# rojas-diego/tokengeex

Hardware: AMD Instinct MI355X
Metric: MB/s raw bytes encoded (and tokens/s) at 32K/64K vocab, 1/2/4/8 GPUs (higher is better)
Workload: dtype f64

## Files before the change

include/tgx.h:

```cpp
#ifndef TGX_H
#define TGX_H

#include <stddef.h>
#include <stdint.h>

#ifdef __cplusplus
extern "C" {
#endif

#define TGX_ABI_VERSION 1

typedef enum tgx_status {
    TGX_OK = 0,
    TGX_ERR_IO = 1,
    TGX_ERR_JSON = 2,
    TGX_ERR_TOKEN_ID_OOB = 3,
    TGX_ERR_NO_PATH = 4,
    TGX_ERR_DEVICE = 5,
    TGX_ERR_Z_NOT_NORMAL = 6,
    TGX_ERR_INVALID = 7,
    TGX_ERR_UNSUPPORTED = 8
} tgx_status;

#define TGX_MAX_TOKEN_LEN 64
// ... 229 lines not shown

double tgx_sample_u01(uint64_t seed, uint64_t sample, uint64_t pos, uint32_t len);
tgx_status tgx_encode_batch_sample(tgx_model *m, const uint8_t *text, const uint64_t *offs,
                                   uint64_t n_samples, double alpha, uint64_t seed,
                                   double *logz, tgx_result **out);
tgx_status tgx_encode_corpus_sample(tgx_model *m, tgx_corpus *c, double alpha, uint64_t seed,
                                    double *logz, tgx_result **out);

#define TGX_MAX_NBEST 16
tgx_status tgx_encode_batch_nbest(tgx_model *m, const uint8_t *text, const uint64_t *offs, uint64_t n_samples,
                                  uint32_t nbest, double *scores, uint32_t *n_found, tgx_result **out);
tgx_status tgx_encode_corpus_nbest(tgx_model *m, tgx_corpus *c, uint32_t nbest,
                                   double *scores, uint32_t *n_found, tgx_result **out);

tgx_status tgx_count_tokens(tgx_model *m, tgx_corpus *c, uint64_t *freq);

tgx_status tgx_count_pairs(tgx_model *m, tgx_corpus *c, uint64_t **keys, uint64_t **counts,
                           uint64_t *n_pairs);
tgx_status tgx_count_pairs_top(tgx_model *m, tgx_corpus *c, uint64_t max_pairs, uint64_t **keys,
                               uint64_t **counts, uint64_t *n_pairs, uint64_t *n_total);

tgx_status tgx_estep(tgx_model *m, tgx_corpus *c, uint64_t snippet_len, double dropout,
                     uint64_t seed, double *expected, double *logz_sum);

void tgx_free(void *p);
void tgx_pool_trim(int device);
void *tgx_host_alloc(uint64_t bytes);
void tgx_host_free(void *p);

double tgx_digamma(double x);
tgx_status tgx_prune_m_step(const double *expected, const uint8_t *keep, uint32_t vocab_size,
                            uint32_t *out_idx, double *out_score, uint32_t *out_n);
tgx_status tgx_prune_alternatives(const tgx_flat_trie *trie, const uint8_t *bytes, const uint64_t *offs,
                                  const double *scores, uint32_t vocab_size, uint8_t *always_keep,
                                  uint32_t *alt_offs, uint32_t **alt_ids);
tgx_status tgx_model_prune_alternatives(const tgx_model *m, uint8_t *always_keep, uint32_t *alt_offs, uint32_t **alt_ids);
tgx_status tgx_prune_select(const uint64_t *freq, const uint8_t *keep, const uint8_t *always_keep,
                            const uint32_t *alt_offs, const uint32_t *alt_ids, const double *scores,
                            uint32_t vocab_size, uint64_t n_samples, uint32_t pruned_size,
                            uint32_t *out_idx, uint32_t *out_n);

int tgx_last_kernel_times(const tgx_model *m, const char **names, float *ms, int cap);
uint64_t tgx_last_algorithmic_bytes(const tgx_model *m);
uint32_t tgx_last_encode_waves_per_cu(const tgx_model *m);
uint64_t tgx_last_encode_redo_samples(const tgx_model *m);
uint64_t tgx_last_encode_long_samples(const tgx_model *m);
uint64_t tgx_last_estep_pieces(const tgx_model *m);
uint64_t tgx_last_estep_redo(const tgx_model *m);
uint32_t tgx_last_encode_corun_cus(const tgx_model *m);
uint32_t tgx_encode_corun_timeouts(const tgx_model *m);
uint32_t tgx_model_score_values(const tgx_model *m);
uint32_t tgx_last_encode_hot_values(const tgx_model *m);
uint32_t tgx_last_encode_lean_items(const tgx_model *m);

static inline double tgx_dropout_u01(uint64_t seed, uint64_t sample, uint64_t pos, uint32_t len) {
    uint64_t x = seed ^ (sample * 0x9E3779B97F4A7C15ULL) ^ (pos * 0xC2B2AE3D27D4EB4FULL) ^
                 ((uint64_t)len * 0x165667B19E3779F9ULL);
    x ^= x >> 30;
    x *= 0xBF58476D1CE4E5B9ULL;
    x ^= x >> 27;
    x *= 0x94D049BB133111EBULL;
    x ^= x >> 31;
    return (double)(x >> 11) * (1.0 / 9007199254740992.0);
}

#ifdef __cplusplus
}
#endif
#endif
```

tokengeex_amd/_lib.py:

```python
from __future__ import annotations

import ctypes as C
import os

import numpy as np

_HERE = os.path.dirname(os.path.abspath(__file__))
LIB_PATH = os.path.join(_HERE, "libtgx.so")

OK, ERR_IO, ERR_JSON, ERR_TOKEN_ID_OOB, ERR_NO_PATH, ERR_DEVICE, ERR_Z_NOT_NORMAL, ERR_INVALID, \
    ERR_UNSUPPORTED = range(9)
MAX_TOKEN_LEN = 64
MAX_NBEST = 16
ESTEP_SNIPPET_LEN = 81920
NO_ID = 0xFFFFFFFF
LAYOUT_PAD_LEFT, LAYOUT_TRUNC_LEFT, LAYOUT_I64 = 1, 2, 4
FRONT_CRLF = 1
SPAN_CHARS = 8

_vp, _u64, _u32, _i, _d = C.c_void_p, C.c_uint64, C.c_uint32, C.c_int, C.c_double
_pvp, _pu64 = C.POINTER(C.c_void_p), C.POINTER(C.c_uint64)
SYMBOLS = {
    "tgx_last_error": (C.c_char_p, []),
    "tgx_last_error_detail": (None, [_pu64, _pu64, _pu64]),
# ... 15 lines not shown
                                     C.POINTER(C.c_double)]),
    "tgx_flat_trie_stats": (None, [_vp, _pu64, _pu64, C.POINTER(C.c_uint32)]),
    "tgx_flat_trie_copy": (None, [_vp, _vp, _vp, _vp]),
    "tgx_tok_hash_selftest": (_i, [_vp, _vp, _u32, C.POINTER(C.c_uint32), _pu64]),
    "tgx_dropout_u01_host": (_d, [_u64, _u64, _u64, _u32]),
    "tgx_encode_batch": (_i, [_vp, _vp, _vp, _u64, _d, _u64, _pvp]),
    "tgx_encode_batch_host": (_i, [_vp, _vp, _vp, _u64, _d, _u64, _vp, _u64, _vp, _pu64]),
    "tgx_encode_batch_multi": (_i, [_vp, _u32, _vp, _vp, _u64, _d, _u64, _vp, _u64, _vp, _pu64]),
    "tgx_result_num_samples": (_u64, [_vp]),
    "tgx_result_num_tokens": (_u64, [_vp]),
    "tgx_result_ids": (_vp, [_vp]),
    "tgx_result_offsets": (_vp, [_vp]),
    "tgx_result_copy_ids": (_i, [_vp, _vp, _u64]),
    "tgx_result_copy_offsets": (_i, [_vp, _vp, _u64]),
    "tgx_result_ids_device": (_vp, [_vp]),
    "tgx_result_offsets_device": (_vp, [_vp]),
    "tgx_result_free": (None, [_vp]),
    "tgx_corpus_upload": (_i, [_i, _vp, _vp, _u64, _pvp]),
    "tgx_corpus_free": (None, [_vp]),
    "tgx_corpus_num_samples": (_u64, [_vp]),
    "tgx_corpus_num_bytes": (_u64, [_vp]),
    "tgx_encode_corpus": (_i, [_vp, _vp, _d, _u64, _pvp]),
    "tgx_count_tokens": (_i, [_vp, _vp, _vp]),
    "tgx_count_pairs": (_i, [_vp, _vp, _pvp, _pvp, _pu64]),
    "tgx_count_pairs_top": (_i, [_vp, _vp, _u64, _pvp, _pvp, _pu64, _pu64]),
    "tgx_estep": (_i, [_vp, _vp, _u64, _d, _u64, _vp, C.POINTER(C.c_double)]),
    "tgx_split_specials": (_i, [_vp, _vp, _u64, _vp, _vp, _u32, _vp, _pvp, _pvp, _pvp, _pu64]),
    "tgx_pack_segments": (_i, [_vp, _vp, _vp, _vp, _u64, _i, _vp, _vp, _pu64]),
    "tgx_normalize_segments": (_i, [_u32, _vp, _vp, _vp, _u64, _pvp, _pvp]),
    "tgx_unidata_version": (C.c_char_p, []),
    "tgx_assemble_ids": (_i, [_vp, _vp, _u64, _vp, _vp, _u32, _vp, _vp]),
    "tgx_decode_batch": (_i, [_vp, _vp, _u32, _vp, _vp, _u32, _vp, _vp, _u64, _i, _pvp, _vp, _pu64, _pu64]),
    "tgx_utf8_lossy": (_u64, [_vp, _u64, _vp]),
    "tgx_substring_df": (_i, [_i, _vp, _u64, _vp, _vp, _vp, _vp, _u64, _u32, _d, _u64, _pvp, _pvp, _pvp, _pu64, _pu64, _pu64]),
    "tgx_substring_df_top": (_i, [_i, _vp, _u64, _vp, _vp, _vp, _vp, _u64, _u32, _d, _u64, _u64, _pvp, _pvp, _pvp, _pu64, _pu64, _pu64,
                                  _pu64, C.POINTER(C.c_uint32)]),
    "tgx_generate_u01": (_d, [_u64, _u64, _u64]),
    "tgx_free": (None, [_vp]),
    "tgx_pool_trim": (None, [_i]),
    "tgx_host_alloc": (_vp, [_u64]),
    "tgx_host_free": (None, [_vp]),
    "tgx_digamma": (_d, [_d]),
    "tgx_prune_m_step": (_i, [_vp, _vp, _u32, _vp, _vp, C.POINTER(C.c_uint32)]),
    "tgx_prune_alternatives": (_i, [_vp, _vp, _vp, _vp, _u32, _vp, _vp, _pvp]),
    "tgx_model_prune_alternatives": (_i, [_vp, _vp, _vp, _pvp]),
    "tgx_prune_select": (_i, [_vp, _vp, _vp, _vp, _vp, _vp, _u32, _u64, _u32, _vp, C.POINTER(C.c_uint32)]),
    "tgx_last_kernel_times": (_i, [_vp, C.POINTER(C.c_char_p), C.POINTER(C.c_float), _i]),
    "tgx_last_algorithmic_bytes": (_u64, [_vp]),
    "tgx_last_encode_waves_per_cu": (_u32, [_vp]),
    "tgx_last_encode_redo_samples": (_u64, [_vp]),
    "tgx_model_score_values": (_u32, [_vp]),
    "tgx_last_encode_hot_values": (_u32, [_vp]),
    "tgx_last_encode_lean_items": (_u32, [_vp]),
    "tgx_last_encode_long_samples": (_u64, [_vp]),
    "tgx_last_estep_pieces": (_u64, [_vp]),
    "tgx_last_estep_redo": (_u64, [_vp]),
    "tgx_last_encode_corun_cus": (_u32, [_vp]),
    "tgx_encode_corun_timeouts": (_u32, [_vp]),
    "tgx_sample_u01": (_d, [_u64, _u64, _u64, _u32]),
    "tgx_encode_batch_sample": (_i, [_vp, _vp, _vp, _u64, _d, _u64, _vp, _pvp]),
    "tgx_encode_corpus_sample": (_i, [_vp, _vp, _d, _u64, _vp, _pvp]),
    "tgx_encode_batch_nbest": (_i, [_vp, _vp, _vp, _u64, _u32, _vp, _vp, _pvp]),
    "tgx_encode_corpus_nbest": (_i, [_vp, _vp, _u32, _vp, _vp, _pvp]),
    "tgx_result_device": (_i, [_vp]),
    "tgx_result_layout_info": (_i, [_vp, _u32, _u32, _pu64, _pu64]),
    "tgx_result_pad_device": (_i, [_vp, _u32, _u32, _u32, _u32, _u32, _vp, _vp, _vp, _vp, _pu64]),
    "tgx_result_pack_device": (_i, [_vp, _u32, _u32, _u32, _u32, _u32, _vp, _vp, _vp, _vp, _pu64]),
    "tgx_layout_pad_host": (_i, [_vp, _vp, _u64, _u32, _u32, _u32, _u32, _u32, _vp, _vp, _vp, _pu64]),
    "tgx_layout_pack_host": (_i, [_vp, _vp, _u64, _u32, _u32, _u32, _u32, _u32, _vp, _vp, _vp, _pu64]),
    "tgx_assemble_result": (_i, [_vp, _vp, _vp, _vp, _u64, _u32, _pvp]),
    "tgx_result_vocab_size": (_u32, [_vp]),
    "tgx_assemble_host": (_i, [_vp, _vp, _u64, _vp, _vp, _u64, _u32, _u32, _vp, _u64, _vp]),
    "tgx_decode_result": (_i, [_vp, _vp, _vp, _vp, _u32, _i, _vp, _pvp, _pu64, _pu64]),
    "tgx_decode_padded": (_i, [_vp, _vp, _u64, _u64, _u32, _vp, _vp, _u32, _vp, _vp, _u32, _i, _vp, _pvp, _pu64, _pu64]),
    "tgx_text_num_rows": (_u64, [_vp]),
    "tgx_text_num_bytes": (_u64, [_vp]),
    "tgx_text_num_replaced": (_u64, [_vp]),
    "tgx_text_device": (_i, [_vp]),
    "tgx_text_copy_bytes": (_i, [_vp, _vp, _u64]),
    "tgx_text_copy_offsets": (_i, [_vp, _vp, _u64]),
    "tgx_text_bytes_device": (_vp, [_vp]),
    "tgx_text_offsets_device": (_vp, [_vp]),
    "tgx_text_free": (None, [_vp]),
    "tgx_corpus_from_text": (_i, [_vp, _pvp]),
    "tgx_decode_rows_host": (_i, [_vp, _vp, _u32, _vp, _vp, _u32, _vp, _u32, _vp, _u64, _u64, _vp, _vp, _u32, _i, _pvp, _vp, _pu64,
                                  _pu64, _pu64]),
    "tgx_result_spans_device": (_i, [_vp, _vp, _vp, _vp, _u32, _u32, _vp, _vp]),
    "tgx_result_pad_spans_device": (_i, [_vp, _vp, _vp, _vp, _u32, _u32, _u32, _u32, _u32, _vp, _vp]),
    "tgx_spans_host": (_i, [_vp, _vp, _u32, _vp, _vp, _u32, _vp, _vp, _u64, _u32, _u32, _u32, _u32, _vp]),
    "tgx_result_window_info": (_i, [_vp, _u32, _u32, _u32, _u32, _u32, _pu64]),
    "tgx_result_window_pad_device": (_i, [_vp, _u32, _u32, _u32, _u32, _u32, _u32, _vp, _u64, _vp, _vp, _vp, _vp, _vp]),
    "tgx_result_window_spans_device": (_i, [_vp, _vp, _vp, _vp, _u32, _u32, _u32, _u32, _u32, _u32, _vp, _u64, _vp]),
    "tgx_layout_windows_host": (_i, [_vp, _vp, _u64, _u32, _u32, _u32, _u32, _u32, _u32, _u64, _vp, _vp, _vp, _vp, _vp, _pu64]),
    "tgx_window_spans_host": (_i, [_vp, _vp, _u32, _vp, _vp, _u32, _vp, _vp, _u64, _u32, _u32, _u32, _u32, _u32, _u64, _vp, _pu64]),
    "tgx_corpus_split_specials": (_i, [_vp, _vp, _vp, _u32, _u32, _pvp, _pvp]),
    "tgx_plan_num_samples": (_u64, [_vp]),
    "tgx_plan_num_segments": (_u64, [_vp]),
    "tgx_plan_num_encoded": (_u64, [_vp]),
    "tgx_plan_device": (_i, [_vp]),
    "tgx_plan_copy": (_i, [_vp, _vp, _u64, _vp, _u64]),
    "tgx_plan_free": (None, [_vp]),
    "tgx_assemble_result_plan": (_i, [_vp, _vp, _vp, _u32, _pvp]),
    "tgx_front_last_times": (_i, [C.POINTER(C.c_char_p), C.POINTER(C.c_float), _i]),
    "tgx_corpus_copy_text": (_i, [_vp, _vp, _u64]),
    "tgx_corpus_copy_offsets": (_i, [_vp, _vp, _u64]),
    "tgx_front_host": (_i, [_vp, _vp, _u64, _vp, _vp, _u32, _u32, _vp, _pvp, _pu64, _pvp, _pvp, _pu64]),
# ... 1042 lines not shown
        ka = np.ctypeslib.as_array(C.cast(keys, C.POINTER(C.c_uint64)), shape=(max(k, 1),))[:k].copy()
        ca = np.ctypeslib.as_array(C.cast(counts, C.POINTER(C.c_uint64)), shape=(max(k, 1),))[:k].copy()
        lib.tgx_free(keys)
        lib.tgx_free(counts)
        return ka, ca, tot.value

    def estep(self, corpus: NativeCorpus, snippet_len: int = ESTEP_SNIPPET_LEN, dropout: float = 0.0,
              seed: int = 0, expected: np.ndarray | None = None) -> tuple[np.ndarray, float]:
        if expected is None:
            expected = np.zeros(self.vocab_size, np.float64)
        assert expected.dtype == np.float64 and expected.shape[0] == self.vocab_size
        z = C.c_double()
        check(lib.tgx_estep(self._h, corpus._h, snippet_len, float(dropout), seed & (2**64 - 1),
                            ptr(expected), C.byref(z)))
        return expected, z.value

    def common_prefix_search(self, s: bytes) -> list[tuple[int, int]]:
        buf = np.frombuffer(s, dtype=np.uint8)
        cap = len(s) + 1
        ids, lens = np.zeros(cap, np.uint32), np.zeros(cap, np.uint32)
        cnt = C.c_uint64()
        check(lib.tgx_common_prefix_search(self._h, ptr(buf) if len(s) else None, len(s), ptr(ids),
                                           ptr(lens), cap, C.byref(cnt)))
        return [(int(ids[i]), int(lens[i])) for i in range(cnt.value)]

    def last_kernel_times(self) -> dict[str, float]:
        names = (C.c_char_p * 8)()
        ms = (C.c_float * 8)()
        n = lib.tgx_last_kernel_times(self._h, names, ms, 8)
        return {names[i].decode(): float(ms[i]) for i in range(n)}

    def last_algorithmic_bytes(self) -> int:
        return lib.tgx_last_algorithmic_bytes(self._h)

    def last_encode_waves_per_cu(self) -> int:
        return lib.tgx_last_encode_waves_per_cu(self._h)

    def last_encode_redo_samples(self) -> int:
        return lib.tgx_last_encode_redo_samples(self._h)

    def score_values(self) -> int:
        return lib.tgx_model_score_values(self._h)

    def last_encode_hot_values(self) -> int:
        return lib.tgx_last_encode_hot_values(self._h)

    def last_encode_lean_items(self) -> tuple[int, int]:
        v = lib.tgx_last_encode_lean_items(self._h)
        return v & 0xFF, (v >> 8) & 0xFF

    def last_encode_lean_step(self) -> bool:
        return bool(self.last_encode_lean_items()[0] & 1)

    def last_encode_long_samples(self) -> int:
        return lib.tgx_last_encode_long_samples(self._h)

    def last_estep_pieces(self) -> int:
        return lib.tgx_last_estep_pieces(self._h)

    def last_estep_redo(self) -> int:
        return lib.tgx_last_estep_redo(self._h)

    def last_encode_corun_cus(self) -> int:
        return lib.tgx_last_encode_corun_cus(self._h)

    def encode_corun_timeouts(self) -> int:
        return lib.tgx_encode_corun_timeouts(self._h)


class FlatTrie:

    def __init__(self, tokens: list[bytes], scores):
        flat, offs = pack(tokens)
        sc = np.ascontiguousarray(scores, dtype=np.float64)
        h = C.c_void_p()
        check(lib.tgx_flat_trie_build(ptr(flat) if flat.size else None, ptr(offs), ptr(sc), len(tokens),
                                      C.byref(h)))
        self._h = h
        self._flat, self._offs, self._sc = flat, offs, sc

    def common_prefix_search8(self, s: bytes, max_hot: int = 6600):
        buf = np.frombuffer(s, dtype=np.uint8)
        cap = len(s) + 1
        ids, lens = np.zeros(cap, np.uint32), np.zeros(cap, np.uint32)
        nh, nc, cov = C.c_uint32(), C.c_uint64(), C.c_double()
        k = lib.tgx_flat_trie_search8(self._h, ptr(self._flat) if self._flat.size else None, ptr(self._offs), ptr(self._sc),
                                      max_hot, ptr(buf) if len(s) else None, len(s), ptr(ids), ptr(lens), cap,
                                      C.byref(nh), C.byref(nc), C.byref(cov))
        if k == 2**64 - 1:
            raise TokenGeeXError("8-byte records need fewer than 2^23 slots")
        return [(int(ids[i]), int(lens[i])) for i in range(k)], {"n_hot": nh.value, "n_cold": nc.value, "hot_coverage": cov.value}

    def __del__(self):
        if getattr(self, "_h", None):
            lib.tgx_flat_trie_free(self._h)
            self._h = None

    def common_prefix_search(self, s: bytes) -> list[tuple[int, int]]:
        buf = np.frombuffer(s, dtype=np.uint8)
        cap = len(s) + 1
        ids, lens = np.zeros(cap, np.uint32), np.zeros(cap, np.uint32)
        k = lib.tgx_flat_trie_search(self._h, ptr(buf) if len(s) else None, len(s), ptr(ids), ptr(lens), cap)
        return [(int(ids[i]), int(lens[i])) for i in range(k)]

    def stats(self) -> dict:
        a, b, c = C.c_uint64(), C.c_uint64(), C.c_uint32()
# ... 88 lines not shown
```

tokengeex_amd/build.py:

```python
from __future__ import annotations

import os
import shutil
import subprocess
import sys

HERE = os.path.dirname(os.path.abspath(__file__))
CSRC = os.path.join(HERE, "csrc")
OUT = os.path.join(HERE, "libtgx.so")
SOURCES = ["kernels.hip", "estep.hip", "encode2.hip", "encode4l.hip", "encode5.hip", "estep4.hip", "estep4l.hip", "estep7.hip", "cuts.hip", "pairs.hip", "generate.hip", "sample.hip", "nbest.hip", "layout.hip", "assemble.hip", "fim.hip", "decode.hip", "spans.hip", "front.hip", "norm.hip", "tgx_api.cpp", "host_twins.cpp", "trie_build.cpp", "prune_host.cpp", "frontback.cpp", "unicode_norm.cpp"]
HEADERS = ["api_internal.h", "kernels.h", "sample.h", "nbest.h", "layout.h", "assemble.h", "fim.h", "decode.h", "spans.h", "front.h", "norm.h", "device_common.h", "lean_gate.h", "trace_body.h", "trie_build.h", "unicode_tables.h", os.path.join("..", "..", "include", "tgx.h")]
ARCH = "gfx950"


def _hipcc() -> str:
    for cand in (os.environ.get("HIPCC"), shutil.which("hipcc"), "/opt/rocm/bin/hipcc"):
        if cand and os.path.exists(cand):
            return cand
    raise RuntimeError("hipcc not found")


def needs_build() -> bool:
    if not os.path.exists(OUT):
        return True
    t = os.path.getmtime(OUT)
    deps = [os.path.join(CSRC, f) for f in SOURCES + HEADERS] + [os.path.abspath(__file__)]
    return any(os.path.getmtime(d) > t for d in deps)


SYNTH_OUT = os.path.join(HERE, "libtgx_synth.so")


def build_synth(force: bool = False) -> str:
    src = os.path.join(CSRC, "synth_gen.c")
    if not force and os.path.exists(SYNTH_OUT) and os.path.getmtime(SYNTH_OUT) >= os.path.getmtime(src):
        return SYNTH_OUT
    subprocess.check_call(["gcc", "-O2", "-std=c11", "-fPIC", "-shared", "-o", SYNTH_OUT + ".tmp", src, "-lm"])
    os.replace(SYNTH_OUT + ".tmp", SYNTH_OUT)
    return SYNTH_OUT


FAST_OUT = os.path.join(HERE, "_tgxfast.so")


def build_pyfast(force: bool = False) -> str:
    import sysconfig
    src = os.path.join(CSRC, "pyfast.c")
    if not force and os.path.exists(FAST_OUT) and os.path.getmtime(FAST_OUT) >= os.path.getmtime(src):
        return FAST_OUT
    inc = sysconfig.get_paths()["include"]
    subprocess.check_call(["gcc", "-O2", "-std=c11", "-fPIC", "-shared", "-pthread", "-I", inc, "-o", FAST_OUT + ".tmp", src])
    os.replace(FAST_OUT + ".tmp", FAST_OUT)
    return FAST_OUT


def build(force: bool = False, verbose: bool = False) -> str:
    from concurrent.futures import ThreadPoolExecutor
    build_synth(force)
    build_pyfast(force)
    if not force and not needs_build():
        return OUT
    objdir = os.path.join(CSRC, "build")
    os.makedirs(objdir, exist_ok=True)
    hdr_time = max(os.path.getmtime(os.path.join(CSRC, h)) for h in HEADERS)
# ... 33 lines not shown
```

tokengeex_amd/csrc/device_common.h:

```cpp
#pragma once
#include <hip/hip_runtime.h>
#include <stdint.h>

namespace tgx {

__device__ __forceinline__ uint32_t readlane_u32(uint32_t v, uint32_t lane) {
    return (uint32_t)__builtin_amdgcn_readlane((int)v, (int)lane);
}
__device__ __forceinline__ uint64_t readlane_u64(uint64_t v, uint32_t lane) {
    uint32_t lo = readlane_u32((uint32_t)v, lane);
    uint32_t hi = readlane_u32((uint32_t)(v >> 32), lane);
    return ((uint64_t)hi << 32) | lo;
}
__device__ __forceinline__ double readlane_f64(double v, uint32_t lane) {
    return __longlong_as_double((long long)readlane_u64((uint64_t)__double_as_longlong(v), lane));
}
__device__ __forceinline__ uint64_t first_u64(uint64_t v) {
    uint32_t lo = (uint32_t)__builtin_amdgcn_readfirstlane((int)(uint32_t)v);
    uint32_t hi = (uint32_t)__builtin_amdgcn_readfirstlane((int)(uint32_t)(v >> 32));
    return ((uint64_t)hi << 32) | lo;
}
__device__ __forceinline__ uint64_t rotl64(uint64_t x, uint32_t r) {
    r &= 63u;
    return (x << r) | (x >> ((64u - r) & 63u));
// ... 98 lines not shown
    return ((uint64_t)hi << 32) | lo;
}

__device__ __forceinline__ uint64_t claim_rows(unsigned long long* queue, bool need_new, uint32_t r) {
    const uint64_t want = __builtin_amdgcn_ballot_w64(need_new) & kRowLane0;
    uint64_t k = ~0ull;
    if (want != 0) {
        const uint64_t base = wave_fetch_add(queue, (uint32_t)__builtin_popcountll(want));
        if (need_new) k = base + (uint64_t)__builtin_popcountll(want & ((1ull << (r * 16u)) - 1ull));
    }
    return k;
}

__device__ __forceinline__ uint64_t claim_rows_chunk(unsigned long long* queue, bool need_new, uint32_t r, uint32_t chunk) {
    const uint64_t want = __builtin_amdgcn_ballot_w64(need_new) & kRowLane0;
    uint64_t k = ~0ull;
    if (want != 0) {
        const uint64_t base = wave_fetch_add(queue, (uint32_t)__builtin_popcountll(want) * chunk);
        if (need_new) k = base + (uint64_t)__builtin_popcountll(want & ((1ull << (r * 16u)) - 1ull)) * chunk;
    }
    return k;
}

__device__ __forceinline__ uint4 load_rec(const uint4* __restrict__ trie, uint32_t t) {
    uint4 r = trie[t];
    asm volatile("" : "+v"(r.x), "+v"(r.y), "+v"(r.z), "+v"(r.w));
    return r;
}

__device__ __forceinline__ uint64_t bp8_base(uint64_t beg, uint32_t s) { return (beg + 128ull * s) & ~3ull; }
__device__ __forceinline__ uint32_t bp8_perm(uint32_t j) { return (j & ~63u) | ((j & 15u) << 2) | ((j >> 4) & 3u); }


constexpr uint32_t kNoStep = 0xFFu;

template <int U>
__device__ __forceinline__ void relax4_step(double sv, double& acc, uint32_t& bpv, uint32_t& fin, uint32_t& fhi) {
    constexpr uint64_t MU = kRowLane0 << U;
    const double best = row_bcast_f64<U>(acc);
    fin = sel_u32(MU, bpv, fin);
    fhi = sel_u32(MU, (uint32_t)((uint64_t)__double_as_longlong(acc) >> 32), fhi);
    const double cand = best + sv;
    const uint64_t take = __builtin_amdgcn_fcmp(cand, acc, 2 ) | MU;
    acc = sel_f64(take, cand, acc);
    bpv = sel_imm_u32<U>(take, bpv);
}

constexpr int kLeanStep = 1, kLeanBcast = 2, kLeanFetch = 4;
constexpr uint32_t kLeanResetHi = 0xFFEFFFFFu;
constexpr uint32_t kLeanUnreachedHi = 0xFFE00000u;
template <int LN>
__device__ __forceinline__ bool relax5_reached(uint32_t fhi) { return (LN & kLeanStep) ? fhi < kLeanUnreachedHi : fhi != 0xFFF00000u; }

template <int U, int LN = 0>
__device__ __forceinline__ void relax5_step(double sv, double& acc, uint32_t& bpv, uint32_t& fin, uint32_t& fhi) {
    constexpr uint64_t MU = kRowLane0 << U;
    double best;
    if constexpr ((LN & kLeanBcast) != 0) best = row_bcast_f64_b<U>(acc);
    else best = row_bcast_f64<U>(acc);
    fin = sel_u32(MU, bpv, fin);
    fhi = sel_u32(MU, (uint32_t)((uint64_t)__double_as_longlong(acc) >> 32), fhi);
    const double acc_r = sel_f64(MU, -__builtin_huge_val(), acc);
    const double cand = best + sv;
    const uint64_t take = __builtin_amdgcn_fcmp(cand, acc_r, 2 );
    asm("v_max_f64 %0, %1, %2" : "=v"(acc) : "v"(acc_r), "v"(cand));
    bpv = sel_imm_u32<U>(take, bpv);
}

template <int U, int LN>
__device__ __forceinline__ void relax5_lean_step(double sv, double& acc, uint32_t& bpv, uint32_t& fin) {
    constexpr uint64_t MU = kRowLane0 << U;
    double best;
    if constexpr ((LN & kLeanBcast) != 0) best = row_bcast_f64_b<U>(acc);
    else best = row_bcast_f64<U>(acc);
    fin = sel_u32(MU, bpv, fin);
    const uint64_t ab = (uint64_t)__double_as_longlong(acc);
    const uint32_t hi_r = sel_u32(MU, kLeanResetHi, (uint32_t)(ab >> 32));
    const double acc_r = __hiloint2double((int)hi_r, (int)(uint32_t)ab);
    const double cand = best + sv;
    const uint64_t take = __builtin_amdgcn_fcmp(cand, acc_r, 2 );
    asm("v_max_f64 %0, %1, %2" : "=v"(acc) : "v"(acc_r), "v"(cand));
    bpv = sel_imm_u32<U>(take, bpv);
}


__device__ __forceinline__ uint32_t rotl32_dev(uint32_t x, int r) { return __builtin_rotateleft32(x, (uint32_t)r); }
__device__ __forceinline__ uint64_t tok_hash64_dev(uint32_t w0, uint32_t w1, uint32_t w2, uint32_t w3, uint32_t len, uint32_t seed) {
    uint32_t a = (w0 ^ (len << 27) ^ seed) * 0x85EBCA6Bu;
    a ^= a >> 15;
    uint32_t b = a;
    a = (a + w1) * 0xC2B2AE35u;
    a ^= a >> 13;
    b = rotl32_dev(b, 11) ^ a;
    a = (a + w2) * 0x27D4EB2Fu;
    a ^= a >> 16;
    b = rotl32_dev(b, 11) ^ a;
    a = (a + w3) * 0x165667B1u;
    a ^= a >> 15;
    b = rotl32_dev(b, 11) + (w0 ^ rotl32_dev(w1, 8) ^ rotl32_dev(w2, 16) ^ rotl32_dev(w3, 24));
    return ((uint64_t)b << 32) | a;
}


__device__ __forceinline__ uint64_t tok_hash64_long_dev(const uint32_t* w, uint32_t len, uint32_t seed) {
    uint32_t a = (w[0] ^ (len << 27) ^ seed) * 0x85EBCA6Bu;
    a ^= a >> 15;
    uint32_t b = a;
    a = (a + w[1]) * 0xC2B2AE35u;
    a ^= a >> 13;
    b = rotl32_dev(b, 11) ^ a;
    a = (a + w[2]) * 0x27D4EB2Fu;
    a ^= a >> 16;
    b = rotl32_dev(b, 11) ^ a;
    a = (a + w[3]) * 0x165667B1u;
    a ^= a >> 15;
    b = rotl32_dev(b, 11) + (w[0] ^ rotl32_dev(w[1], 8) ^ rotl32_dev(w[2], 16) ^ rotl32_dev(w[3], 24));
    if (len > 16u) {
        a = (a + w[4]) * 0x85EBCA6Bu;
        a ^= a >> 15;
        b = rotl32_dev(b, 11) ^ a;
        a = (a + w[5]) * 0xC2B2AE35u;
        a ^= a >> 13;
        b = rotl32_dev(b, 11) ^ a;
        a = (a + w[6]) * 0x27D4EB2Fu;
        a ^= a >> 16;
        b = rotl32_dev(b, 11) ^ a;
        a = (a + w[7]) * 0x165667B1u;
        a ^= a >> 15;
        b = rotl32_dev(b, 11) + (w[4] ^ rotl32_dev(w[5], 8) ^ rotl32_dev(w[6], 16) ^ rotl32_dev(w[7], 24));
    }
    return ((uint64_t)b << 32) | a;
}


__device__ __forceinline__ int row_max_exponent(double acc) {
// ... 20 lines not shown
```

tokengeex_amd/csrc/encode5.hip:

```cpp
#include <hip/hip_runtime.h>
#include <stdint.h>

#include <type_traits>

#include "device_common.h"
#include "kernels.h"

namespace tgx {

constexpr uint32_t kE5RowStride = 512;
constexpr uint32_t kE5GroupBytes = 4 * kE5RowStride;

template <int PPL>
struct WalkCtx {
    __amdgpu_buffer_rsrc_t trie;
    uint32_t s, l32;
    double dropout;
    uint64_t seed;
    bool estep_rule = false;
};

struct Res5 {
    __amdgpu_buffer_rsrc_t cold;
    uint32_t tab;
// ... 223 lines not shown
    fval = sel_f64(MU, acc, fval);
    const double best = row_bcast_f64<U>(acc);
    const double cur = sel_f64(MU, far, acc);
    const uint32_t curbp = sel_u32(MU, fbp, bpv);
    far = sel_f64(MU, -__builtin_huge_val(), far);
    const double cand = best + sv;
    const uint64_t take = __builtin_amdgcn_fcmp(cand, cur, 2 );
    asm("v_max_f64 %0, %1, %2" : "=v"(acc) : "v"(cur), "v"(cand));
    bpv = sel_imm_u32<U>(take, curbp);
}

template <bool DROPOUT>
__device__ __forceinline__ void e5_long_tail(__amdgpu_buffer_rsrc_t trie, const uint8_t* __restrict__ text16, uint32_t rec_x, bool alive,
                                             uint32_t maxd, uint32_t lane, uint32_t g, uint32_t list_off, double dropout, uint64_t seed,
                                             uint32_t s, uint32_t pg) {
    bool more = alive && maxd > 16u;
    if (__builtin_amdgcn_ballot_w64(more) == 0) return;
    struct __attribute__((packed, aligned(1))) Bytes16 { uint32_t w[4]; };
    Bytes16 b{{0u, 0u, 0u, 0u}};
    if (more) b = *reinterpret_cast<const Bytes16*>(text16);
    uint32_t x = rec_x;
#pragma unroll 1
    for (uint32_t d = 16u; d < 32u; ++d) {
        more = more && d < maxd;
        if (__builtin_amdgcn_ballot_w64(more) == 0) break;
        const uint32_t bi = d - 16u;
        const uint32_t word = (bi & 8u) ? ((bi & 4u) ? b.w[3] : b.w[2]) : ((bi & 4u) ? b.w[1] : b.w[0]);
        const uint32_t c = (word >> ((bi & 3u) * 8u)) & 0xFFu;
        const uint2 rec = buf_ld8(trie, more ? ((x ^ (c << 3)) & 0xFFFFFFu) : 0u);
        more = more && (rec.x >> 24) == c;
        const uint32_t rank = rec.y & 0xFFFFu;
        bool term = more && rank != 0u;
        if (DROPOUT) {
            if (term) term = dropout < dropout_u01(seed, s, pg, d + 1u);
        }
        if (term) {
            const uint32_t slot = __hip_atomic_fetch_add((__attribute__((address_space(3))) uint32_t*)(uintptr_t)list_off, 1u, __ATOMIC_RELAXED, __HIP_MEMORY_SCOPE_WORKGROUP);
            if (slot < kE5LongCap) lds_st<uint32_t>(list_off + 8u + slot * 4u, lane | (g << 6) | (d << 8) | (rank << 16));
        }
        x = rec.x;
    }
}

#define E5_STAMP(i)                                                    \
    if (P.stamps) {                                                    \
        __builtin_amdgcn_sched_barrier(0);                             \
        const uint64_t _now = (uint64_t)__builtin_amdgcn_s_memtime(); \
        __builtin_amdgcn_s_waitcnt(0xC07F);                            \
        __builtin_amdgcn_sched_barrier(0);                             \
        seg[i] += _now - t_last;                                       \
        t_last = _now;                                                 \
    }

template <bool DROPOUT, bool COLD, int PPL, bool LONG, int CK = 0, int LN = 0>
__global__ __launch_bounds__(1024, (PPL == 1 ? 8 : (PPL == 2 ? 6 : (PPL == 3 ? 4 : 1)))) void encode5_kernel(EncodeParams P, Encode5Params Q) {
    static_assert(!LONG || PPL == 4, "the long-token build runs four positions per lane");
    static_assert(LN == 0 || (!LONG && !DROPOUT), "the long-token and dropout builds keep the kernel as it was");
    extern __shared__ __align__(16) unsigned char smem[];
    constexpr uint32_t LM = LONG ? 32 : 16;
    constexpr uint32_t SPAN = 16u * PPL;
    const uint32_t lane = threadIdx.x & 63u;
    const uint32_t l = lane & 15u, r = lane >> 4;
    const uint32_t wave = threadIdx.x >> 6;
    const uint2* __restrict__ trie = reinterpret_cast<const uint2*>(Q.trie8);
    const __amdgpu_buffer_rsrc_t trie_b = make_rsrc(Q.trie8, Q.trie_bytes);
    const uint32_t lds0 = (uint32_t)reinterpret_cast<uintptr_t>(smem);
    double* const score_tab = reinterpret_cast<double*>(smem);
    const uint32_t hot_bytes = 8u * (Q.n_hot + 1u);
    const __amdgpu_buffer_rsrc_t values = make_rsrc(reinterpret_cast<const unsigned char*>(Q.values) + hot_bytes, 8u * (Q.n_values - Q.n_hot));
    const uint2* rootc = reinterpret_cast<const uint2*>(smem + Q.root_off);
    unsigned char* wbase = smem + Q.idx_off + (size_t)wave * (PPL * kE5GroupBytes);
    {
        for (uint32_t i = threadIdx.x; i <= Q.n_hot; i += blockDim.x) score_tab[i] = Q.values[i];
        uint2* rw = reinterpret_cast<uint2*>(smem + Q.root_off);
        for (uint32_t i = threadIdx.x; i < 256u; i += blockDim.x) rw[i] = trie[(Q.root_base & ~255u) + i];
        if (Q.started && threadIdx.x == 0u) __hip_atomic_fetch_add(Q.started, 1u, __ATOMIC_RELAXED, __HIP_MEMORY_SCOPE_SYSTEM);
        __syncthreads();
    }
    const __amdgpu_buffer_rsrc_t cold_values = values;

    uint32_t s = 0, n = 0, p0 = 0;
    uint64_t beg = 0;
    bool live = false, need_new = true;
    const double ninf = -__builtin_huge_val();
    double acc = ninf, far = ninf;
    uint32_t bpv = kNoStep, fbp = kFarCode;
    bool redo = false;
    uint32_t wn[4 * PPL + 1];
    uint32_t pk = 0, pk_j = 0;
    bool pk_dirty = false;
#pragma unroll
    for (int q = 0; q <= 4 * PPL; ++q) wn[q] = 0;
    const uint32_t my_col = r * kE5RowStride + ((l - 1u) & 15u) * 32u;
    const uint32_t wbase_off = lds0 + Q.idx_off + wave * (PPL * kE5GroupBytes);
    const uint32_t wr_off = wbase_off + r * kE5RowStride + l * 2u;
    const uint32_t col_off = wbase_off + my_col;
    const uint32_t list_off = lds0 + Q.list_off + wave * ((kE5LongBytes + 15u) & ~15u);
    uint64_t seg[5] = {0, 0, 0, 0, 0};
    uint64_t t_last = P.stamps ? (uint64_t)__builtin_amdgcn_s_memtime() : 0;
    uint32_t iters = 0;

    uint64_t local_next = 0, local_end = 0;
    for (;;) {
        {
            uint64_t k = ~0ull;
            const bool have_local = need_new && local_next < local_end;
            if (have_local) k = local_next++;
            const uint64_t kc = claim_rows_chunk(P.queue, need_new && !have_local, r, Q.claim_chunk);
            if (need_new && !have_local) {
                k = kc;
// ... 120 lines not shown
                    n_list = (uint32_t)__builtin_amdgcn_readfirstlane((int)lds_ld<uint32_t>(list_off));
                    slow = n_list != 0u || __builtin_amdgcn_ballot_w64((uint32_t)((uint64_t)__double_as_longlong(far) >> 32) != 0xFFF00000u) != 0;
                }
                if (LONG && slow) {
                    auto rank_of = [&](int u) { return (u & 1) ? (cw[u >> 1] >> 16) : (cw[u >> 1] & 0xFFFFu); };
                    double fval = ninf;
                    relax5l_step<0>(e5_score_one<COLD>(lds0, cold_values, rank_of(0), hot_bytes), acc, bpv, far, fbp, fin[g], fval);
                    relax5l_step<1>(e5_score_one<COLD>(lds0, cold_values, rank_of(1), hot_bytes), acc, bpv, far, fbp, fin[g], fval);
                    relax5l_step<2>(e5_score_one<COLD>(lds0, cold_values, rank_of(2), hot_bytes), acc, bpv, far, fbp, fin[g], fval);
                    relax5l_step<3>(e5_score_one<COLD>(lds0, cold_values, rank_of(3), hot_bytes), acc, bpv, far, fbp, fin[g], fval);
                    relax5l_step<4>(e5_score_one<COLD>(lds0, cold_values, rank_of(4), hot_bytes), acc, bpv, far, fbp, fin[g], fval);
                    relax5l_step<5>(e5_score_one<COLD>(lds0, cold_values, rank_of(5), hot_bytes), acc, bpv, far, fbp, fin[g], fval);
                    relax5l_step<6>(e5_score_one<COLD>(lds0, cold_values, rank_of(6), hot_bytes), acc, bpv, far, fbp, fin[g], fval);
                    relax5l_step<7>(e5_score_one<COLD>(lds0, cold_values, rank_of(7), hot_bytes), acc, bpv, far, fbp, fin[g], fval);
                    relax5l_step<8>(e5_score_one<COLD>(lds0, cold_values, rank_of(8), hot_bytes), acc, bpv, far, fbp, fin[g], fval);
                    relax5l_step<9>(e5_score_one<COLD>(lds0, cold_values, rank_of(9), hot_bytes), acc, bpv, far, fbp, fin[g], fval);
                    relax5l_step<10>(e5_score_one<COLD>(lds0, cold_values, rank_of(10), hot_bytes), acc, bpv, far, fbp, fin[g], fval);
                    relax5l_step<11>(e5_score_one<COLD>(lds0, cold_values, rank_of(11), hot_bytes), acc, bpv, far, fbp, fin[g], fval);
                    relax5l_step<12>(e5_score_one<COLD>(lds0, cold_values, rank_of(12), hot_bytes), acc, bpv, far, fbp, fin[g], fval);
                    relax5l_step<13>(e5_score_one<COLD>(lds0, cold_values, rank_of(13), hot_bytes), acc, bpv, far, fbp, fin[g], fval);
                    relax5l_step<14>(e5_score_one<COLD>(lds0, cold_values, rank_of(14), hot_bytes), acc, bpv, far, fbp, fin[g], fval);
                    relax5l_step<15>(e5_score_one<COLD>(lds0, cold_values, rank_of(15), hot_bytes), acc, bpv, far, fbp, fin[g], fval);
                    const uint32_t cnt = n_list < kE5LongCap ? n_list : kE5LongCap;
#pragma unroll 1
                    for (uint32_t i = 0; i < cnt; ++i) {
                        const uint32_t e = (uint32_t)__builtin_amdgcn_readfirstlane((int)lds_ld<uint32_t>(list_off + 8u + i * 4u));
                        if (((e >> 6) & 3u) != (uint32_t)g) continue;
                        const uint32_t src = e & 63u, d = (e >> 8) & 31u;
                        const double score = e5_score_one<COLD>(lds0, cold_values, e >> 16, hot_bytes);
                        const double cand = readlane_f64(fval, src) + score;
                        const uint32_t tt = (src & 15u) + d + 1u;
                        const bool mine = (lane >> 4) == (src >> 4) && l == (tt & 15u);
                        const bool to_far = tt >= 32u;
                        const double curv = to_far ? far : acc;
                        const uint32_t curc = to_far ? fbp : bpv;
                        const bool longer = !(curc & kFarCode) || d > (curc & 31u);
                        const bool take = mine && (cand > curv || (cand == curv && longer));
                        if (take && to_far) {
                            far = cand;
                            fbp = kFarCode | d;
                        }
                        if (take && !to_far) {
                            acc = cand;
                            bpv = kFarCode | d;
                        }
                    }
                    reached[g] = fval > ninf;
                    if (g + 1 < PPL) {
                        load_iw(g + 1, nw);
                        if (!COLD) e5_scores_issue<4>(lds0, nw, 0, sa);
                    }
                    continue;
                }
                if constexpr (LN == 0) {
                    if (COLD) {
                        double sv[8], sw[8];
                        e5_scores_cold<8>(lds0, cold_values, cw, 0, hot_bytes, sv);
                        e5_scores_cold<8>(lds0, cold_values, cw, 8, hot_bytes, sw);
                        if (g + 1 < PPL) load_iw(g + 1, nw);
                        relax5_step<0>(sv[0], acc, bpv, fin[g], fhi);
                        relax5_step<1>(sv[1], acc, bpv, fin[g], fhi);
                        relax5_step<2>(sv[2], acc, bpv, fin[g], fhi);
                        relax5_step<3>(sv[3], acc, bpv, fin[g], fhi);
                        relax5_step<4>(sv[4], acc, bpv, fin[g], fhi);
                        relax5_step<5>(sv[5], acc, bpv, fin[g], fhi);
                        relax5_step<6>(sv[6], acc, bpv, fin[g], fhi);
                        relax5_step<7>(sv[7], acc, bpv, fin[g], fhi);
                        relax5_step<8>(sw[0], acc, bpv, fin[g], fhi);
                        relax5_step<9>(sw[1], acc, bpv, fin[g], fhi);
                        relax5_step<10>(sw[2], acc, bpv, fin[g], fhi);
                        relax5_step<11>(sw[3], acc, bpv, fin[g], fhi);
                        relax5_step<12>(sw[4], acc, bpv, fin[g], fhi);
                        relax5_step<13>(sw[5], acc, bpv, fin[g], fhi);
                        relax5_step<14>(sw[6], acc, bpv, fin[g], fhi);
                        relax5_step<15>(sw[7], acc, bpv, fin[g], fhi);
                    } else {
                        e5_scores_issue<4>(lds0, cw, 4, sb);
                        if (g + 1 < PPL) load_iw(g + 1, nw);
                        relax5_step<0>(e5_score_value(sa[0]), acc, bpv, fin[g], fhi);
                        relax5_step<1>(e5_score_value(sa[1]), acc, bpv, fin[g], fhi);
                        relax5_step<2>(e5_score_value(sa[2]), acc, bpv, fin[g], fhi);
                        relax5_step<3>(e5_score_value(sa[3]), acc, bpv, fin[g], fhi);
                        e5_scores_issue<4>(lds0, cw, 8, sa);
                        relax5_step<4>(e5_score_value(sb[0]), acc, bpv, fin[g], fhi);
                        relax5_step<5>(e5_score_value(sb[1]), acc, bpv, fin[g], fhi);
                        relax5_step<6>(e5_score_value(sb[2]), acc, bpv, fin[g], fhi);
                        relax5_step<7>(e5_score_value(sb[3]), acc, bpv, fin[g], fhi);
                        e5_scores_issue<4>(lds0, cw, 12, sb);
                        relax5_step<8>(e5_score_value(sa[0]), acc, bpv, fin[g], fhi);
                        relax5_step<9>(e5_score_value(sa[1]), acc, bpv, fin[g], fhi);
                        relax5_step<10>(e5_score_value(sa[2]), acc, bpv, fin[g], fhi);
                        relax5_step<11>(e5_score_value(sa[3]), acc, bpv, fin[g], fhi);
                        if (g + 1 < PPL) e5_scores_issue<4>(lds0, nw, 0, sa);
                        relax5_step<12>(e5_score_value(sb[0]), acc, bpv, fin[g], fhi);
                        relax5_step<13>(e5_score_value(sb[1]), acc, bpv, fin[g], fhi);
                        relax5_step<14>(e5_score_value(sb[2]), acc, bpv, fin[g], fhi);
                        relax5_step<15>(e5_score_value(sb[3]), acc, bpv, fin[g], fhi);
                    }
                    reached[g] = fhi != 0xFFF00000u;
                } else {
                    const bool full = !(LN & kLeanStep) || ((end_groups >> g) & 1u) != 0u;
#define E5_STEP(U, SV)                                                   \
        if (FULL) relax5_step<U, LN>(SV, acc, bpv, fin[g], fhi);              \
        else relax5_lean_step<U, LN>(SV, acc, bpv, fin[g]);
                    auto steps = [&](auto full_tag) {
                        constexpr bool FULL = decltype(full_tag)::value;
                        if (COLD) {
                            double sv[8], sw[8];
                            e5_scores_cold<8, LN>(lds0, cold_values, cw, 0, hot_bytes, sv);
                            e5_scores_cold<8, LN>(lds0, cold_values, cw, 8, hot_bytes, sw);
                            if (g + 1 < PPL) load_iw(g + 1, nw);
                            E5_STEP(0, sv[0]) E5_STEP(1, sv[1]) E5_STEP(2, sv[2]) E5_STEP(3, sv[3])
                            E5_STEP(4, sv[4]) E5_STEP(5, sv[5]) E5_STEP(6, sv[6]) E5_STEP(7, sv[7])
                            E5_STEP(8, sw[0]) E5_STEP(9, sw[1]) E5_STEP(10, sw[2]) E5_STEP(11, sw[3])
                            E5_STEP(12, sw[4]) E5_STEP(13, sw[5]) E5_STEP(14, sw[6]) E5_STEP(15, sw[7])
                        } else {
                            e5_scores_issue<4, LN>(lds0, cw, 4, sb);
                            if (g + 1 < PPL) load_iw(g + 1, nw);
                            E5_STEP(0, e5_score_value(sa[0])) E5_STEP(1, e5_score_value(sa[1]))
                            E5_STEP(2, e5_score_value(sa[2])) E5_STEP(3, e5_score_value(sa[3]))
                            e5_scores_issue<4, LN>(lds0, cw, 8, sa);
                            E5_STEP(4, e5_score_value(sb[0])) E5_STEP(5, e5_score_value(sb[1]))
                            E5_STEP(6, e5_score_value(sb[2])) E5_STEP(7, e5_score_value(sb[3]))
                            e5_scores_issue<4, LN>(lds0, cw, 12, sb);
                            E5_STEP(8, e5_score_value(sa[0])) E5_STEP(9, e5_score_value(sa[1]))
                            E5_STEP(10, e5_score_value(sa[2])) E5_STEP(11, e5_score_value(sa[3]))
                            if (g + 1 < PPL) e5_scores_issue<4, LN>(lds0, nw, 0, sa);
                            E5_STEP(12, e5_score_value(sb[0])) E5_STEP(13, e5_score_value(sb[1]))
                            E5_STEP(14, e5_score_value(sb[2])) E5_STEP(15, e5_score_value(sb[3]))
                        }
                    };
                    if (full) steps(std::true_type{});
                    else steps(std::false_type{});
#undef E5_STEP
                    reached[g] = !full || relax5_reached<LN>(fhi);
                }
            }
        } else {
#pragma unroll
            for (int g = 0; g < PPL; ++g) {
                fin[g] = kNoStep;
                reached[g] = true;
            }
        }
        __builtin_amdgcn_wave_barrier();
        if (!(P.flags & 32u)) __builtin_amdgcn_s_setprio(2);
        E5_STAMP(3)

        uint8_t* const bpw = P.bp8 + bp8_base(beg, s);
#pragma unroll
        for (int g = 0; g < PPL; ++g)
            if (live && pg[g] >= 1u && pg[g] <= n) {
                const uint32_t b = reached[g] ? (LONG ? e5_winner_len_m1(fin[g], l) : ((l - fin[g] - 1u) & 15u)) : 0xFFu;
                const uint32_t j = pg[g] - 1u, kq = (j >> 4) & 3u;
                pk = (kq == 0u) ? b : (pk | (b << (8u * kq)));
                pk_j = j;
                pk_dirty = true;
                if (kq == 3u) {
                    __builtin_nontemporal_store(pk, reinterpret_cast<uint32_t*>(bpw + (bp8_perm(j) & ~3u)));
                    pk_dirty = false;
                }
            }
        if (LONG) {
            const uint32_t n_all = (uint32_t)__builtin_amdgcn_readfirstlane((int)lds_ld<uint32_t>(list_off));
            if (n_all > kE5LongCap) {
                if (live && !redo && l == 0u) P.redo_list[atomicAdd(P.redo_count, 1ULL)] = s;
                redo = true;
            }
        }
        if (live && n - p0 < SPAN && pk_dirty) {
            __builtin_nontemporal_store(pk, reinterpret_cast<uint32_t*>(bpw + (bp8_perm(pk_j) & ~3u)));
            pk_dirty = false;
        }
        if (live) {
            const uint32_t left = n - p0;
            if (left < SPAN) {
#pragma unroll
                for (int g = 0; g < PPL; ++g)
                    if (left == 16u * g + l) P.status[s] = (n == 0u || reached[g]) ? 1u : 0u;
                need_new = true;
            } else {
                p0 += SPAN;
            }
        }
        E5_STAMP(4)
    }
    if (P.stamps && lane == 0) {
        unsigned long long* o = P.stamps + (size_t)(blockIdx.x * (blockDim.x >> 6) + wave) * 8u;
        for (int i = 0; i < 5; ++i) o[i] = seg[i];
        o[5] = iters;
    }
}

constexpr uint32_t kE6Walkers = 3;
constexpr uint32_t kE6Slots = kE6Walkers + 2u;
struct E6Ctrl {
    uint32_t epoch;
    uint32_t s, n, trip0;
    uint64_t beg;
    uint32_t relax_done;
    uint32_t pad_;
    uint32_t walk_done[8];
    uint32_t ack[4];
    uint32_t pool_used[8];
    uint32_t pad2_[4];
};
constexpr uint32_t kE6Done = 0xFFFFFFFFu;

__device__ __forceinline__ uint32_t lds_load(const uint32_t* p) { return __hip_atomic_load(p, __ATOMIC_RELAXED, __HIP_MEMORY_SCOPE_WORKGROUP); }
__device__ __forceinline__ void lds_store(uint32_t* p, uint32_t v) { __hip_atomic_store(p, v, __ATOMIC_RELAXED, __HIP_MEMORY_SCOPE_WORKGROUP); }

template <bool COLD, int LN = 0>
__device__ __forceinline__ void e6_load_quarter(uint32_t tab, __amdgpu_buffer_rsrc_t cold, uint32_t hot_bytes,
                                                const uint32_t (&iw)[8], int q, double (&sv)[4]) {
    if (COLD) {
        e5_scores_cold<4, LN>(tab, cold, iw, 4 * q, hot_bytes, sv);
    } else {
        u32x2_t sp[4];
        e5_scores_issue<4, LN>(tab, iw, 4 * q, sp);
#pragma unroll
        for (int u = 0; u < 4; ++u) sv[u] = e5_score_value(sp[u]);
    }
}

template <bool DROPOUT, bool COLD, int LN = 0>
__global__ __launch_bounds__(64 * (1 + 4 * kE6Walkers), 8) void encode6_kernel(EncodeParams P, Encode5Params Q) {
    static_assert(LN == 0 || !DROPOUT, "the dropout builds keep the kernel as it was");
    static_assert((LN & (kLeanStep | kLeanBcast)) == 0, "encode6_kernel: the score fetch only (the lean step spills here)");
    extern __shared__ __align__(16) unsigned char smem[];
    constexpr uint32_t LM = 16;
    constexpr uint32_t K = kE6Walkers, G = kE6Slots;
    const uint32_t lane = threadIdx.x & 63u;
// ... 418 lines not shown
        if (live) {
            if (n - p0 < SPAN) need_new = true;
            else p0 += SPAN;
        }
    }
    if (zsum != 0.0) atomicAdd(P.logz_sum, zsum);
}

typedef void (*estep5_fn)(Estep4Params, Encode5Params);
static estep5_fn pick_estep5(bool dropout, bool cold, int ppl) {
#define TGX_E5F(D, C)                                                                        \
    (ppl == 1 ? estep5_fwd_kernel<D, C, 1> : ppl == 2 ? estep5_fwd_kernel<D, C, 2> : ppl == 3 ? estep5_fwd_kernel<D, C, 3> : estep5_fwd_kernel<D, C, 4>)
    if (dropout) return cold ? TGX_E5F(true, true) : TGX_E5F(true, false);
    return cold ? TGX_E5F(false, true) : TGX_E5F(false, false);
#undef TGX_E5F
}
hipError_t estep5_waves_per_simd(bool dropout, bool cold, int ppl, int* out) {
    hipFuncAttributes attr;
    hipError_t e = hipFuncGetAttributes(&attr, reinterpret_cast<const void*>(pick_estep5(dropout, cold, ppl)));
    if (e != hipSuccess) return e;
    const int regs = (attr.numRegs + 7) & ~7;
    *out = regs > 0 ? (512 / regs > 8 ? 8 : 512 / regs) : 8;
    return hipSuccess;
}
hipError_t launch_estep5_fwd(const Estep4Params& p, Encode5Params q, bool cold, int ppl, int waves, uint32_t blocks, hipStream_t stream) {
    const uint32_t lds = encode5_lds_layout(q.n_hot, false, waves, ppl, &q.list_off, &q.root_off, &q.idx_off);
    if (lds > 160u * 1024u || q.n_hot > q.n_values || (!cold && q.n_hot != q.n_values) || ppl < 1 || ppl > 4) return hipErrorInvalidValue;
    estep5_fn fn = pick_estep5(p.dropout > 0.0, cold, ppl);
    hipError_t e = hipFuncSetAttribute(reinterpret_cast<const void*>(fn), hipFuncAttributeMaxDynamicSharedMemorySize, 160 * 1024);
    if (e != hipSuccess) return e;
    hipLaunchKernelGGL(fn, dim3(blocks), dim3(64u * (uint32_t)waves), lds, stream, p, q);
    return hipGetLastError();
}

typedef void (*encode5_fn)(EncodeParams, Encode5Params);
#ifdef TGX_E5_LEAN_ITEMS
constexpr int kE5LeanHot = TGX_E5_LEAN_ITEMS, kE5LeanCold = TGX_E5_LEAN_ITEMS, kE5LeanCold3 = TGX_E5_LEAN_ITEMS;
constexpr int kE6Lean = kLeanFetch;
#else
constexpr int kE5LeanHot = kLeanFetch;
constexpr int kE5LeanCold = kLeanFetch;
constexpr int kE5LeanCold3 = kLeanStep | kLeanBcast | kLeanFetch;
constexpr int kE6Lean = kLeanFetch;
#endif
static_assert(kE5LeanHot > 0 && kE5LeanHot <= 7 && kE5LeanCold > 0 && kE5LeanCold <= 7 && kE5LeanCold3 > 0 && kE5LeanCold3 <= 7,
              "a mask of kLeanStep, kLeanBcast, kLeanFetch");
constexpr int lean_without_step(int items) { return items & ~kLeanStep; }
bool encode5_has_lean(bool dropout, bool long_tokens) { return !dropout && !long_tokens; }
int encode5_lean_items(bool cold, int ppl, bool step_ok) {
    const int items = cold ? (ppl == 3 ? kE5LeanCold3 : kE5LeanCold) : kE5LeanHot;
    return step_ok ? items : lean_without_step(items);
}
int encode6_lean_items() { return kE6Lean; }
static encode5_fn pick_encode5(bool dropout, bool cold, int ppl, bool long_tokens, int compact, bool lean, bool step_ok) {
    if (long_tokens) {
        if (cold) return dropout ? encode5_kernel<true, true, 4, true> : encode5_kernel<false, true, 4, true>;
        return dropout ? encode5_kernel<true, false, 4, true> : encode5_kernel<false, false, 4, true>;
    }
    if (dropout) {
        if (cold) {
            if (ppl == 1) return encode5_kernel<true, true, 1, false>;
            if (ppl == 2) return encode5_kernel<true, true, 2, false>;
            if (ppl == 3) return encode5_kernel<true, true, 3, false>;
            return encode5_kernel<true, true, 4, false>;
        }
        if (ppl == 1) return encode5_kernel<true, false, 1, false>;
        if (ppl == 2) return encode5_kernel<true, false, 2, false>;
        if (ppl == 3) return encode5_kernel<true, false, 3, false>;
        return encode5_kernel<true, false, 4, false>;
    }
#define TGX_E5K(C, PL, LN) \
    (compact == 4 ? encode5_kernel<false, C, PL, false, 4, LN> : compact == 5 ? encode5_kernel<false, C, PL, false, 5, LN> \
     : compact == 6 ? encode5_kernel<false, C, PL, false, 6, LN> : compact == 7 ? encode5_kernel<false, C, PL, false, 7, LN> \
     : compact == 8 ? encode5_kernel<false, C, PL, false, 8, LN> : encode5_kernel<false, C, PL, false, 0, LN>)
#define TGX_E5L(LNH, LNC, LNC3) \
    if (cold) { \
        if (ppl == 1) return encode5_kernel<false, true, 1, false, 0, LNC>; \
        if (ppl == 2) return TGX_E5K(true, 2, LNC); \
        if (ppl == 3) return TGX_E5K(true, 3, LNC3); \
        return TGX_E5K(true, 4, LNC); \
    } \
    if (ppl == 1) return encode5_kernel<false, false, 1, false, 0, LNH>; \
    if (ppl == 2) return TGX_E5K(false, 2, LNH); \
    if (ppl == 3) return TGX_E5K(false, 3, LNH); \
    return TGX_E5K(false, 4, LNH);
    if (lean && step_ok) {
        TGX_E5L(kE5LeanHot, kE5LeanCold, kE5LeanCold3)
    }
    if (lean) {
        TGX_E5L(lean_without_step(kE5LeanHot), lean_without_step(kE5LeanCold), lean_without_step(kE5LeanCold3))
    }
    TGX_E5L(0, 0, 0)
#undef TGX_E5L
#undef TGX_E5K
}

uint32_t encode5_lds_layout(uint32_t n_hot, bool long_tokens, int waves, int ppl, uint32_t* list_off, uint32_t* root_off, uint32_t* idx_off) {
    const uint32_t lo = (8u * (n_hot + 1u) + 15u) & ~15u;
    const uint32_t score_bytes = lo + (long_tokens ? (uint32_t)waves * ((kE5LongBytes + 15u) & ~15u) : 0u);
    if (list_off) *list_off = lo;
    const uint32_t ro = (score_bytes + 15u) & ~15u;
    const uint32_t io = (ro + 2048u + 511u) & ~511u;
    if (root_off) *root_off = ro;
    if (idx_off) *idx_off = io;
    return io + (uint32_t)waves * (uint32_t)ppl * kE5GroupBytes;
}
uint32_t encode5_max_hot(bool long_tokens, int waves, int ppl, uint32_t budget) {
    const uint32_t fixed = encode5_lds_layout(0u, long_tokens, waves, ppl, nullptr, nullptr, nullptr) + 512u;
    return budget > fixed + 64u ? (budget - fixed) / 8u : 0u;
}

hipError_t encode5_waves_per_simd(bool dropout, bool cold, int ppl, bool long_tokens, int compact, bool lean, bool step_ok, int* out) {
    hipFuncAttributes attr;
    hipError_t e = hipFuncGetAttributes(&attr, reinterpret_cast<const void*>(pick_encode5(dropout, cold, ppl, long_tokens, compact, lean && encode5_has_lean(dropout, long_tokens), step_ok)));
    if (e != hipSuccess) return e;
    const int regs = (attr.numRegs + 7) & ~7;
    *out = regs > 0 ? (512 / regs > 8 ? 8 : 512 / regs) : 8;
    return hipSuccess;
}

uint32_t encode6_lds_layout(uint32_t n_hot, uint32_t pool, uint32_t* root_off, uint32_t* ctrl_off, uint32_t* ring_off) {
    const uint32_t score_bytes = 8u * (1u + 4u * kE6Slots * pool + n_hot);
    const uint32_t ro = (score_bytes + 15u) & ~15u;
    const uint32_t co = ro + 2048u;
    const uint32_t go = (co + 4u * (uint32_t)sizeof(E6Ctrl) + 511u) & ~511u;
    if (root_off) *root_off = ro;
    if (ctrl_off) *ctrl_off = co;
    if (ring_off) *ring_off = go;
    return go + 4u * kE6Slots * kE5GroupBytes;
}
uint32_t encode6_pool_total(uint32_t pool) { return 4u * kE6Slots * pool; }
uint32_t encode6_max_hot(uint32_t budget, uint32_t pool) {
    const uint32_t fixed = encode6_lds_layout(0u, pool, nullptr, nullptr, nullptr) + 512u;
    return budget > fixed + 64u ? (budget - fixed) / 8u : 0u;
}
static hipError_t lean_lds_check(const void* fn) {
    hipFuncAttributes attr;
    const hipError_t e = hipFuncGetAttributes(&attr, fn);
    if (e != hipSuccess) return e;
    return attr.sharedSizeBytes == 0 ? hipSuccess : hipErrorInvalidValue;
}

hipError_t launch_encode6(const EncodeParams& p, Encode5Params q, bool cold, bool lean, uint32_t blocks, hipStream_t stream) {
    q.ring_slots = kE6Slots;
    if (!cold) q.pool = 0u;
    const uint32_t lds = encode6_lds_layout(q.n_hot, q.pool, &q.root_off, &q.ctrl_off, &q.ring_off);
    if (lds > 160u * 1024u || q.n_hot > q.n_values || (!cold && q.n_hot != q.n_values) ||
        (uint64_t)q.n_values + 4ull * kE6Slots * q.pool > 65535ull)
        return hipErrorInvalidValue;
    lean = lean && encode5_has_lean(p.dropout > 0.0, false);
    auto fn = cold ? (p.dropout > 0.0 ? encode6_kernel<true, true> : lean ? encode6_kernel<false, true, kE6Lean> : encode6_kernel<false, true>)
                   : (p.dropout > 0.0 ? encode6_kernel<true, false> : lean ? encode6_kernel<false, false, kE6Lean> : encode6_kernel<false, false>);
    hipError_t e = hipFuncSetAttribute(reinterpret_cast<const void*>(fn), hipFuncAttributeMaxDynamicSharedMemorySize, 160 * 1024);
    if (e != hipSuccess) return e;
    if (lean && (e = lean_lds_check(reinterpret_cast<const void*>(fn))) != hipSuccess) return e;
    hipLaunchKernelGGL(fn, dim3(blocks), dim3(64u * (1u + 4u * kE6Walkers)), lds, stream, p, q);
    return hipGetLastError();
}

hipError_t launch_encode5(const EncodeParams& p, Encode5Params q, bool cold, int ppl, bool long_tokens, int compact, bool lean, bool step_ok,
                          int waves, uint32_t blocks, uint32_t min_lds, hipStream_t stream) {
    uint32_t lds = encode5_lds_layout(q.n_hot, long_tokens, waves, ppl, &q.list_off, &q.root_off, &q.idx_off);
    if (lds > 160u * 1024u || q.n_hot > q.n_values || (!cold && q.n_hot != q.n_values) || (long_tokens && ppl != 4) ||
        (compact != 0 && (compact < 4 || compact > 8)))
        return hipErrorInvalidValue;
    lean = lean && encode5_has_lean(p.dropout > 0.0, long_tokens);
    encode5_fn fn = pick_encode5(p.dropout > 0.0, cold, ppl, long_tokens, compact, lean, step_ok);
    hipError_t e = hipFuncSetAttribute(reinterpret_cast<const void*>(fn), hipFuncAttributeMaxDynamicSharedMemorySize, 160 * 1024);
    if (e != hipSuccess) return e;
    if (lean && (e = lean_lds_check(reinterpret_cast<const void*>(fn))) != hipSuccess) return e;
    if (lds < min_lds && min_lds <= 160u * 1024u) lds = min_lds;
    hipLaunchKernelGGL(fn, dim3(blocks), dim3(64u * (uint32_t)waves), lds, stream, p, q);
    return hipGetLastError();
}

}
```

tokengeex_amd/csrc/kernels.h:

```cpp
#pragma once
#include <hip/hip_runtime.h>
#include <stdint.h>

#include "decode.h"
#include "fim.h"
#include "spans.h"

namespace tgx {

constexpr uint32_t kTraceStride = 2;

struct EncodeParams {
    const uint8_t* text;
    const uint64_t* offs;
    const uint32_t* order;
    uint64_t n_samples;
    const void* trie;
    const uint32_t* tokid;
    uint32_t root_base;
    uint32_t n_slots;
    uint32_t lm;
    uint32_t* bp;
    uint32_t* tmp;
    uint32_t* counts;
// ... 184 lines not shown
    uint32_t n_slots;
    uint32_t root_base;
    const double* wtab;
    uint32_t n_tok, n_hot;
    double* expected;
    double* zsnip;
    double* logz_sum;
    unsigned long long* range_flag;
    unsigned long long* queue;
    double* alpha;
    int32_t* aexp;
    unsigned char* mscratch;
    double dropout;
    uint64_t seed;
    uint32_t root_off, zero_off, idx_off;
};
uint32_t estep7_redo_max_hot(bool wide);
hipError_t launch_estep7_redo(Estep7RedoParams p, bool wide, uint32_t num_cus, hipStream_t stream);
uint32_t estep7_lds_layout(uint32_t n_hot, bool wide, int waves, int ppl, uint32_t* root_off, uint32_t* zero_off, uint32_t* idx_off);
uint32_t estep7_max_hot(bool wide, int waves, int ppl, uint32_t budget);
hipError_t estep7_waves_per_simd(bool dropout, bool cold, bool wide, int ppl, int* out);
hipError_t launch_estep7(Estep7Params p, bool wide, int ppl, int waves, uint32_t blocks, hipStream_t stream);
hipError_t launch_match_count(const uint8_t* text, uint64_t n_bytes, uint32_t chunk, uint64_t stride, const void* trie8t, uint32_t n_slots,
                              uint32_t root_base, uint32_t n_tok, unsigned int* counts, uint32_t num_cus, hipStream_t stream);
hipError_t launch_value_count(const uint8_t* text, uint64_t n_bytes, uint32_t chunk, uint64_t stride, const void* trie8, uint32_t n_slots,
                              uint32_t root_base, uint32_t n_values, uint32_t max_len, unsigned int* counts, uint32_t num_cus, hipStream_t stream);
hipError_t launch_rank_remap(void* trie8t, uint32_t n_slots, const uint32_t* perm, hipStream_t stream);
hipError_t launch_snip_z_check(const double* zsnip, uint64_t n_snips, unsigned long long* err_snip, hipStream_t stream);
hipError_t launch_piece_z_add(const double* zarr, const uint32_t* psnip, const uint32_t* order, uint64_t n_order, double* zsnip, hipStream_t stream);

hipError_t estep4_prepare();
hipError_t launch_estep4_fwd(const Estep4Params& p, uint32_t num_cus, hipStream_t stream);
hipError_t launch_estep4_bwd(const Estep4Params& p, uint32_t num_cus, hipStream_t stream);
hipError_t estep4l_prepare();
hipError_t launch_estep4l_fwd(const Estep4Params& p, int ppl, bool long_tokens, uint32_t num_cus, hipStream_t stream);
hipError_t launch_estep4l_bwd(const Estep4Params& p, int ppl, bool long_tokens, uint32_t num_cus, uint32_t groups_wanted, hipStream_t stream);
hipError_t launch_estep4_reduce(const double* rep, double* out, uint32_t n_slots, uint32_t n_replicas,
                                hipStream_t stream);

uint32_t estep_lds_bytes_per_block(uint32_t lm);
uint32_t estep_waves_per_block(uint32_t lm);
hipError_t estep_max_blocks_per_cu(uint32_t lm, int* out);
hipError_t launch_estep(const EstepParams& p, uint32_t blocks, hipStream_t stream);

uint32_t encode_lds_bytes_per_block(uint32_t lm);
uint32_t encode_waves_per_block(uint32_t lm);
hipError_t encode_max_blocks_per_cu(uint32_t lm, int* out);
hipError_t launch_encode(const EncodeParams& p, uint32_t blocks, hipStream_t stream);
uint32_t encode4_group_bytes();
hipError_t encode4_waves_per_simd(bool dropout, int ppl, bool root, int* out);
hipError_t launch_encode4(const EncodeParams& p, int ppl, int waves, uint32_t blocks, bool root, hipStream_t stream);
uint32_t encode4_lds_bytes(int waves, int ppl, bool root);
hipError_t launch_trace(const EncodeParams& p, uint32_t blocks, hipStream_t stream);
uint32_t encode5_lds_layout(uint32_t n_hot, bool long_tokens, int waves, int ppl, uint32_t* list_off, uint32_t* root_off, uint32_t* idx_off);
uint32_t encode5_max_hot(bool long_tokens, int waves, int ppl, uint32_t budget);
bool encode5_has_lean(bool dropout, bool long_tokens);
int encode5_lean_items(bool cold, int ppl, bool step_ok);
int encode6_lean_items();
hipError_t encode5_waves_per_simd(bool dropout, bool cold, int ppl, bool long_tokens, int compact, bool lean, bool step_ok, int* out);
uint32_t encode6_lds_layout(uint32_t n_hot, uint32_t pool, uint32_t* root_off, uint32_t* ctrl_off, uint32_t* ring_off);
uint32_t encode6_max_hot(uint32_t budget, uint32_t pool);
uint32_t encode6_pool_total(uint32_t pool);
hipError_t estep5_waves_per_simd(bool dropout, bool cold, int ppl, int* out);
hipError_t launch_estep5_fwd(const struct Estep4Params& p, Encode5Params q, bool cold, int ppl, int waves, uint32_t blocks, hipStream_t stream);
hipError_t launch_encode6(const EncodeParams& p, Encode5Params q, bool cold, bool lean, uint32_t blocks, hipStream_t stream);
hipError_t launch_encode5(const EncodeParams& p, Encode5Params q, bool cold, int ppl, bool long_tokens, int compact, bool lean, bool step_ok,
                          int waves, uint32_t blocks, uint32_t min_lds, hipStream_t stream);
hipError_t launch_encode2(const EncodeParams& p, uint32_t num_cus, bool permuted, hipStream_t stream);
hipError_t launch_trace32(const EncodeParams& p, uint32_t blocks, bool permuted, hipStream_t stream);
hipError_t launch_encode4l(const EncodeParams& p, uint32_t num_cus, hipStream_t stream);
hipError_t scan_temp_bytes(uint64_t n, size_t* bytes);
hipError_t launch_scan(uint32_t* counts, uint64_t* offsets, uint64_t n, void* temp, size_t temp_bytes, hipStream_t stream);
hipError_t launch_compact(const CompactParams& p, uint32_t blocks, bool rows, hipStream_t stream);

struct LayoutParams {
    const uint32_t* ids;
    const uint64_t* offs;
    uint64_t n_rows;
    uint32_t len;
    uint32_t pad, bos, eos;
    uint32_t flags;
    void* out;
    uint8_t* mask;
    int32_t* lengths;
    int32_t* doc;
    int32_t* pos;
    unsigned long long* counter;
};
hipError_t launch_layout_max_row(const uint64_t* offs, uint64_t n_rows, unsigned long long* max_out, hipStream_t stream);
hipError_t launch_layout_pad(const LayoutParams& p, hipStream_t stream);
hipError_t launch_layout_pack(const LayoutParams& p, uint64_t n_stream, uint64_t n_out, hipStream_t stream);
struct WindowParams {
    LayoutParams base;
    const uint64_t* wo;
    uint32_t stride;
    int32_t* window_row;
    int32_t* window_first;
};
hipError_t launch_layout_window_count(const uint64_t* offs, uint64_t n_rows, uint32_t room, uint32_t step, uint32_t* counts,
                                      unsigned long long* max_out, hipStream_t stream);
hipError_t launch_layout_windows(const WindowParams& q, uint64_t n_windows, hipStream_t stream);

struct AssembleParams {
    const uint32_t* ids;
    const uint64_t* offs;
    const uint64_t* seg_offs;
    const int32_t* seg_special;
    uint64_t* rank;
    uint64_t* starts;
    uint64_t n_segs, n_samples;
    uint64_t n_out;
    uint32_t vocab_size;
    uint32_t* out_ids;
    uint64_t* out_offs;
};
hipError_t assemble_scan_temp_bytes(uint64_t n_segs, size_t* bytes);
hipError_t launch_assemble_ranks(int32_t* seg_special, uint64_t* rank, uint64_t n_segs, void* temp, size_t temp_bytes, hipStream_t stream);
hipError_t launch_assemble_starts(const AssembleParams& p, hipStream_t stream);
hipError_t launch_assemble_fill(const AssembleParams& p, hipStream_t stream);
// ... 64 lines not shown
```

tokengeex_amd/csrc/kernels.hip:

```cpp
#include <hip/hip_runtime.h>
#include <stdint.h>

#include <rocprim/device/device_scan.hpp>
#include <rocprim/iterator/transform_iterator.hpp>

#include "kernels.h"
#include "trace_body.h"
#include "device_common.h"

namespace tgx {

struct WaveCtx {
    const uint4* __restrict__ trie;
    uint32_t root_base;
    double dropout;
    uint64_t seed;
    bool use_dropout;
    uint32_t flags;
};

__device__ __forceinline__ void block_generic(const WaveCtx& C, const uint8_t* __restrict__ text, uint32_t n,
                                              uint32_t s, uint32_t p0, uint32_t lane, uint32_t LM,
                                              double* sc, uint32_t* hl, uint8_t* txt, uint32_t* __restrict__ bp,
                                              double& acc, uint32_t& bpv, uint64_t& reach, uint32_t& reach_n) {
// ... 424 lines not shown
            relax5_step<6>(sv[6], acc, bpv, fin[g], fhi);
            relax5_step<7>(sv[7], acc, bpv, fin[g], fhi);
            relax5_step<8>(sv[8], acc, bpv, fin[g], fhi);
            relax5_step<9>(sv[9], acc, bpv, fin[g], fhi);
            relax5_step<10>(sv[10], acc, bpv, fin[g], fhi);
            relax5_step<11>(sv[11], acc, bpv, fin[g], fhi);
            relax5_step<12>(sv[12], acc, bpv, fin[g], fhi);
            relax5_step<13>(sv[13], acc, bpv, fin[g], fhi);
            relax5_step<14>(sv[14], acc, bpv, fin[g], fhi);
            relax5_step<15>(sv[15], acc, bpv, fin[g], fhi);
            reached[g] = fhi != 0xFFF00000u;
        }
        __builtin_amdgcn_wave_barrier();
        TGX_STAMP(3)

        uint8_t* const bpw = P.bp8 + bp8_base(beg, s);
#pragma unroll
        for (int g = 0; g < PPL; ++g)
            if (live && pg[g] >= 1u && pg[g] <= n) {
                const uint32_t b = reached[g] ? ((l - fin[g] - 1u) & 15u) : 0xFFu;
                const uint32_t j = pg[g] - 1u, kq = (j >> 4) & 3u;
                pk = (kq == 0u) ? b : (pk | (b << (8u * kq)));
                pk_j = j;
                pk_dirty = true;
                if (kq == 3u) {
                    __builtin_nontemporal_store(pk, reinterpret_cast<uint32_t*>(bpw + (bp8_perm(j) & ~3u)));
                    pk_dirty = false;
                }
            }
        if (live && n - p0 < SPAN && pk_dirty) {
            __builtin_nontemporal_store(pk, reinterpret_cast<uint32_t*>(bpw + (bp8_perm(pk_j) & ~3u)));
            pk_dirty = false;
        }
        if (live) {
            const uint32_t left = n - p0;
            if (left < SPAN) {
#pragma unroll
                for (int g = 0; g < PPL; ++g)
                    if (left == 16u * g + l) P.status[s] = (n == 0u || reached[g]) ? 1u : 0u;
                need_new = true;
            } else {
                p0 += SPAN;
            }
        }
        TGX_STAMP(4)
    }
    if (STAMP && lane == 0 && P.stamps) {
        unsigned long long* o = P.stamps + (size_t)(blockIdx.x * wpb + wave) * 8u;
        for (int i = 0; i < 5; ++i) o[i] = seg[i];
        o[5] = iters;
    }
}

template <bool STAMP, bool CARRY, int K>
__global__ __launch_bounds__(256) void trace_kernel(EncodeParams P) {
    __shared__ typename TraceRingEntry<CARRY>::type ring_all[4][kTraceRing];
    trace_body<16, true, STAMP, CARRY, K>(P, ring_all[threadIdx.x >> 6]);
}

__global__ __launch_bounds__(1024) void scan_counts_kernel(const uint32_t* __restrict__ counts,
                                                           uint64_t* __restrict__ offsets,
                                                           uint64_t n) {
    __shared__ uint64_t wsum[16];
    __shared__ uint64_t carry_s;
    constexpr uint32_t E = 8;
    const uint32_t tid = threadIdx.x, lane = tid & 63u, wave = tid >> 6;
    if (tid == 0) carry_s = 0;
    __syncthreads();
    for (uint64_t base = 0; base < n; base += 1024u * E) {
        const uint64_t i0 = base + (uint64_t)tid * E;
        uint32_t c[E];
        uint64_t v = 0;
#pragma unroll
        for (uint32_t e = 0; e < E; ++e) {
            c[e] = (i0 + e < n) ? counts[i0 + e] : 0u;
            v += c[e];
        }
        uint64_t x = v;
        for (int off = 1; off < 64; off <<= 1) {
            uint64_t y = __shfl_up(x, off);
            if ((int)lane >= off) x += y;
        }
        if (lane == 63) wsum[wave] = x;
        __syncthreads();
        uint64_t wprefix = 0;
        for (uint32_t w = 0; w < wave; ++w) wprefix += wsum[w];
        const uint64_t carry = carry_s;
        uint64_t run = carry + wprefix + x - v;
#pragma unroll
        for (uint32_t e = 0; e < E; ++e) {
            if (i0 + e < n) offsets[i0 + e] = run;
            run += c[e];
        }
        __syncthreads();
        if (tid == 1023) carry_s = run;
        __syncthreads();
    }
    if (tid == 0) offsets[n] = carry_s;
}

template <bool ROWS>
__global__ __launch_bounds__(256) void compact_kernel(CompactParams P) {
    const uint32_t lane = threadIdx.x & 63u;
    const uint32_t sub = ROWS ? (lane & 15u) : lane, width = ROWS ? 16u : 64u;
    const uint64_t n_units = (uint64_t)gridDim.x * 4u * (ROWS ? 4u : 1u);
    const uint32_t wave_id = blockIdx.x * 4u + (threadIdx.x >> 6);
    for (uint64_t k = ROWS ? (uint64_t)wave_id * 4u + (lane >> 4) : (uint64_t)wave_id; k < P.n_samples; k += n_units) {
        const uint32_t s = ROWS ? (uint32_t)k : P.order[k];
        const uint64_t end = P.offs[s + 1];
        const uint64_t o0 = P.out_offs[s];
// ... 32 lines not shown
}

hipError_t launch_encode(const EncodeParams& p, uint32_t blocks, hipStream_t stream) {
    const uint32_t lds = encode_lds_bytes_per_block(p.lm);
    const dim3 block(64u * encode_waves_per_block(p.lm));
    hipLaunchKernelGGL(pick_kernel(p.lm), dim3(blocks), block, lds, stream, p);
    return hipGetLastError();
}

hipError_t encode_max_blocks_per_cu(uint32_t lm, int* out) {
    const uint32_t lds = encode_lds_bytes_per_block(lm);
    const int threads = (int)(64u * encode_waves_per_block(lm));
    if (lds > 160u * 1024u) return hipErrorInvalidValue;
    encode_fn fn = pick_kernel(lm);
    hipError_t e = hipFuncSetAttribute(reinterpret_cast<const void*>(fn),
                                       hipFuncAttributeMaxDynamicSharedMemorySize, (int)lds);
    if (e != hipSuccess) return e;
    return hipOccupancyMaxActiveBlocksPerMultiprocessor(out, fn, threads, lds);
}

typedef void (*encode4_fn)(EncodeParams);
static encode4_fn pick_encode4(bool dropout, int ppl, bool stamp, bool root) {
    if (stamp) return encode4_kernel<false, 1, true, false>;
    if (root) return dropout ? encode4_kernel<true, 1, false, true> : encode4_kernel<false, 1, false, true>;
    if (ppl == 1) return dropout ? encode4_kernel<true, 1, false, false> : encode4_kernel<false, 1, false, false>;
    if (ppl == 2) return dropout ? encode4_kernel<true, 2, false, false> : encode4_kernel<false, 2, false, false>;
    return dropout ? encode4_kernel<true, 4, false, false> : encode4_kernel<false, 4, false, false>;
}
uint32_t encode4_group_bytes() { return kRows4GroupBytes; }
uint32_t encode4_lds_bytes(int waves, int ppl, bool root) {
    return (root ? 4096u : 0u) + (uint32_t)waves * (uint32_t)ppl * kRows4GroupBytes;
}
hipError_t encode4_waves_per_simd(bool dropout, int ppl, bool root, int* out) {
    root = root && ppl == 1;
    hipFuncAttributes attr;
    hipError_t e = hipFuncGetAttributes(&attr, reinterpret_cast<const void*>(pick_encode4(dropout, ppl, false, root)));
    if (e != hipSuccess) return e;
    const int regs = (attr.numRegs + 7) & ~7;
    *out = regs > 0 ? (512 / regs > 8 ? 8 : 512 / regs) : 8;
    return hipSuccess;
}
hipError_t launch_encode4(const EncodeParams& p, int ppl, int waves, uint32_t blocks, bool root, hipStream_t stream) {
    const bool stamp = p.stamps != nullptr;
    root = root && !stamp && ppl == 1;
    encode4_fn fn = pick_encode4(p.dropout > 0.0, ppl, stamp, root);
    hipError_t e = hipFuncSetAttribute(reinterpret_cast<const void*>(fn), hipFuncAttributeMaxDynamicSharedMemorySize, 160 * 1024);
    if (e != hipSuccess) return e;
    hipLaunchKernelGGL(fn, dim3(blocks), dim3(64u * (uint32_t)waves), encode4_lds_bytes(waves, stamp ? 1 : ppl, root), stream, p);
    return hipGetLastError();
}
template <bool STAMP, bool CARRY>
static void launch_trace_stride(const EncodeParams& p, uint32_t blocks, hipStream_t stream) {
    switch (p.trace_stride) {
        case 1: hipLaunchKernelGGL((trace_kernel<STAMP, CARRY, 1>), dim3(blocks), dim3(256), 0, stream, p); break;
        case 2: hipLaunchKernelGGL((trace_kernel<STAMP, CARRY, 2>), dim3(blocks), dim3(256), 0, stream, p); break;
        case 3: hipLaunchKernelGGL((trace_kernel<STAMP, CARRY, 3>), dim3(blocks), dim3(256), 0, stream, p); break;
        default: hipLaunchKernelGGL((trace_kernel<STAMP, CARRY, 0>), dim3(blocks), dim3(256), 0, stream, p); break;
    }
}
hipError_t launch_trace(const EncodeParams& p, uint32_t blocks, hipStream_t stream) {
    if (p.stamps)
        launch_trace_stride<true, false>(p, blocks, stream);
    else if (p.trace_carry)
        launch_trace_stride<false, true>(p, blocks, stream);
    else
        launch_trace_stride<false, false>(p, blocks, stream);
    return hipGetLastError();
}

struct WidenU32 {
    __host__ __device__ uint64_t operator()(uint32_t x) const { return (uint64_t)x; }
};
hipError_t scan_temp_bytes(uint64_t n, size_t* bytes) {
    *bytes = 0;
    if (n <= 65536) return hipSuccess;
    auto in = rocprim::make_transform_iterator((const uint32_t*)nullptr, WidenU32());
    return rocprim::exclusive_scan(nullptr, *bytes, in, (uint64_t*)nullptr, (uint64_t)0, (size_t)(n + 1), rocprim::plus<uint64_t>());
}
hipError_t launch_scan(uint32_t* counts, uint64_t* offsets, uint64_t n, void* temp, size_t temp_bytes, hipStream_t stream) {
    if (n <= 65536 || !temp) {
        hipLaunchKernelGGL(scan_counts_kernel, dim3(1), dim3(1024), 0, stream, counts, offsets, n);
        return hipGetLastError();
    }
    hipError_t e = hipMemsetAsync(counts + n, 0, 4, stream);
    if (e != hipSuccess) return e;
    auto in = rocprim::make_transform_iterator((const uint32_t*)counts, WidenU32());
    return rocprim::exclusive_scan(temp, temp_bytes, in, offsets, (uint64_t)0, (size_t)(n + 1), rocprim::plus<uint64_t>(), stream);
}

hipError_t launch_compact(const CompactParams& p, uint32_t blocks, bool rows, hipStream_t stream) {
    if (rows)
        hipLaunchKernelGGL(compact_kernel<true>, dim3(blocks), dim3(256), 0, stream, p);
    else
        hipLaunchKernelGGL(compact_kernel<false>, dim3(blocks), dim3(256), 0, stream, p);
    return hipGetLastError();
}

}
```

tokengeex_amd/csrc/tgx_api.cpp:

```cpp
#include <hip/hip_runtime.h>

#include <algorithm>
#include <unordered_set>
#include <cstdarg>
#include <cstddef>
#include <cstdio>
#include <cstdlib>
#include <cmath>
#include <cstring>
#include <chrono>
#include <condition_variable>
#include <memory>
#include <mutex>
#include <new>
#include <numeric>
#include <string>
#include <thread>
#include <vector>

#include "../../include/tgx.h"
#include "api_internal.h"
#include "assemble.h"
#include "decode.h"
#include "front.h"
#include "kernels.h"
#include "layout.h"
#include "lean_gate.h"
#include "spans.h"
#include "nbest.h"
#include "norm.h"
#include "sample.h"
#include "trie_build.h"

using namespace tgx::host;

tgx_status tgx_set_error(tgx_status st, const char* msg) {
    g_err_msg = msg ? msg : "";
    return st;
}
namespace {

#define HIP_TRY(expr)                                                                     \
    do {                                                                                  \
        hipError_t _e = (expr);                                                           \
        if (_e != hipSuccess)                                                             \
            return fail(TGX_ERR_DEVICE, "HIP error %d (%s) at %s:%d: %s", (int)_e,        \
                        hipGetErrorString(_e), __FILE__, __LINE__, #expr);                \
    } while (0)

struct PoolEntry {
    void* ptr;
    size_t bytes;
    int device;
};
std::mutex g_pool_mu;
std::vector<PoolEntry> g_pool;
size_t g_pool_bytes = 0;
constexpr size_t kPoolMaxBytes = 64ull << 30;

void pool_trim(int device) {
    std::vector<PoolEntry> victims;
    {
        std::lock_guard<std::mutex> lk(g_pool_mu);
        for (size_t i = 0; i < g_pool.size();) {
            if (device < 0 || g_pool[i].device == device) {
                victims.push_back(g_pool[i]);
                g_pool_bytes -= g_pool[i].bytes;
                g_pool.erase(g_pool.begin() + (long)i);
            } else {
                i++;
            }
        }
    }
    if (victims.empty()) return;
    int prev = -1;
    (void)hipGetDevice(&prev);
    for (const PoolEntry& e : victims) {
        (void)hipSetDevice(e.device);
        (void)hipFree(e.ptr);
// ... 131 lines not shown
    unsigned long long err_piece;
};
static_assert(offsetof(DeviceCtrl::Estep, redo_count) == 8 && offsetof(DeviceCtrl::Estep, queue_bwd) == 16 &&
                  offsetof(DeviceCtrl::Estep, range_flag) == 24 && sizeof(DeviceCtrl::Estep) == 32,
              "the E-step words are cleared by one memset");
struct HostCtrl {
    unsigned long long err;
    unsigned long long total_tokens;
};

}

struct tgx_model {
    int device = 0;
    uint32_t vocab_size = 0;
    uint32_t lm = 0;
    bool scores_finite = true;
    tgx::FlatTrie flat;
    void* d_trie = nullptr;
    uint32_t* d_tokid = nullptr;
    DeviceCtrl* d_ctrl = nullptr;
    HostCtrl* h_ctrl = nullptr;
    hipStream_t stream = nullptr;
    hipStream_t stream2 = nullptr;
    hipEvent_t ev_fork = nullptr, ev_join = nullptr;
    unsigned int* h_started = nullptr;
    int num_cus = 0;
    int blocks_per_cu = 0;
    std::vector<uint8_t> vocab_bytes;
    std::vector<uint64_t> vocab_offs;
    std::vector<double> vocab_scores;
    tgx::FlatTrie flat_rev;
    void* d_trie_rev = nullptr;
    bool rev_host_built = false;
    void* d_trie_w = nullptr;
    void* d_trie_rev_w = nullptr;
    uint64_t last_long_samples = 0;
    uint64_t last_estep_pieces = 0;
    uint32_t last_corun_cus = 0;
    double e7_overflow_share = 0.0;
    bool values_ranked = false;
    uint32_t corun_wait_timeouts = 0;
    uint64_t last_redo_samples = 0;
    int last_encode_waves_per_cu = 0;
    bool estep_linear_ok = false;
    tgx::TokHashTable tokhash;
    void* d_tokhash = nullptr;
    void* d_trie8 = nullptr;
    double* d_values = nullptr;
    std::vector<double> value_coverage;
    uint32_t n_values = 0, root_base8 = 0;
    uint32_t last_n_hot = 0;
    bool lean_scores_ok = false;
    uint32_t last_lean_items = 0;
    bool have_trie8 = false;
    bool encode_tables_ready = false;
    bool estep_trie8_tried = false;
    uint64_t estep_calls = 0;
    bool have_wvalues = false;
    double* d_wvalues = nullptr;
    bool tokhash_host_built = false;
    void* d_trie8t = nullptr;
    double* d_wtab = nullptr;
    std::vector<uint32_t> id_of_rank;
    uint32_t n_tok7 = 0, root_base7 = 0;
    bool trie8t_tried = false, have_trie8t = false;
    uint64_t last_estep_redo = 0;
    uint8_t* d_dec_len = nullptr;
    void* d_dec_slots = nullptr;
    uint8_t* d_dec_bytes = nullptr;
    uint64_t* d_dec_offs = nullptr;
    bool decode_tables_ready = false;
    uint16_t* d_span_words = nullptr;
    bool span_words_ready = false;
    int estep_blocks_per_cu = 0;
    KernelTime timed[kMaxTimed] = {};
    int n_timed = 0;
    uint64_t last_alg_bytes = 0;
    std::mutex mu;
};

struct tgx_corpus {
    int device = 0;
    uint64_t n_samples = 0, n_bytes = 0, max_len = 0;
    std::vector<uint64_t> h_offs;
    std::vector<uint32_t> h_sorted_len;
    std::vector<uint64_t> h_sorted_cum;
    PoolBuf<uint8_t> d_text_alloc;
    uint8_t* d_text = nullptr;
    PoolBuf<uint64_t> d_offs;
    PoolBuf<uint32_t> d_order;
    PoolBuf<uint32_t> d_bp, d_tmp, d_counts, d_status;
    PoolBuf<void> d_scan_tmp;
    size_t scan_tmp_bytes = 0;
    struct EstepWork {
        uint64_t snippet_len = 0;
        std::vector<uint64_t> soffs, sbase;
        std::vector<uint32_t> ssample, order;
        PoolBuf<uint64_t> d_soffs, d_sbase;
        PoolBuf<uint32_t> d_order, d_ssample;
        uint32_t window = 0;
        uint64_t n_windows = 0;
        PoolBuf<uint32_t> d_win_snip, d_win_k;
    } es;
    std::mutex mu;
};
// ... 56 lines not shown
    if (hipGetDeviceCount(&n) != hipSuccess) {
        (void)hipGetLastError();
        return 0;
    }
    return n;
}
tgx_status require_device(int* n_devices = nullptr) {
    const int n = usable_device_count();
    if (n_devices) *n_devices = n;
    if (n <= 0) return fail(TGX_ERR_DEVICE, "no usable HIP device (gfx950 required)");
    return TGX_OK;
}

bool debug_on() {
    static int v = -1;
    if (v < 0) {
        const char* e = getenv("TGX_DEBUG");
        v = (e && *e && *e != '0') ? 1 : 0;
    }
    return v == 1;
}

const char* knob(const char* name) {
    static int on = -1;
    if (on < 0) {
        const char* e = getenv("TGX_KNOBS");
        on = ((e && *e && *e != '0') || debug_on()) ? 1 : 0;
    }
    return on == 1 ? getenv(name) : nullptr;
}

void time_begin(tgx_model* m, const char* name) {
    if (debug_on()) {
        fprintf(stderr, "[tgx] launch %s\n", name);
        fflush(stderr);
    }
    if (m->n_timed >= kMaxTimed) return;
    KernelTime& t = m->timed[m->n_timed];
    t.name = name;
    t.used = true;
    (void)hipEventRecord(t.start, m->stream);
}
void time_end(tgx_model* m) {
    if (debug_on()) {
        hipError_t e = hipStreamSynchronize(m->stream);
        fprintf(stderr, "[tgx]   done: %s\n", hipGetErrorString(e));
        fflush(stderr);
    }
    if (m->n_timed >= kMaxTimed) return;
    (void)hipEventRecord(m->timed[m->n_timed].stop, m->stream);
    m->n_timed++;
}

tgx_status ensure_scratch(tgx_corpus* c) {
    HIP_TRY(hipSetDevice(c->device));
    if (!c->d_bp) HIP_TRY(c->d_bp.alloc(c->device, std::max((size_t)c->n_bytes * 4 + 256, (size_t)c->n_bytes + 128 * (size_t)c->n_samples + 512)));
    if (!c->d_counts) HIP_TRY(c->d_counts.alloc(c->device, (size_t)c->n_samples * 4 + 256));
    if (!c->d_status) HIP_TRY(c->d_status.alloc(c->device, (size_t)c->n_samples * 4 + 256));
    if (!c->d_tmp) HIP_TRY(c->d_tmp.alloc(c->device, (size_t)c->n_bytes * 4 + 256));
    return TGX_OK;
}

uint32_t grid_blocks(const tgx_model* m, uint64_t n_samples) {
    const uint64_t wpb = tgx::encode_waves_per_block(m->lm);
    uint64_t want = (n_samples + wpb - 1) / wpb;
    uint64_t cap = (uint64_t)m->num_cus * (uint64_t)std::max(1, m->blocks_per_cu);
    return (uint32_t)std::max<uint64_t>(1, std::min(want, cap));
}

void knob_int(const char* name, int lo, int hi, int* x) {
    if (const char* e = knob(name)) {
        const int v = atoi(e);
        if (v >= lo && v <= hi) *x = v;
    }
}
uint32_t knob_cap_hot(const char* name, uint32_t n_hot) {
    if (const char* e = knob(name)) {
        const int v = atoi(e);
        if (v >= 0) n_hot = std::min(n_hot, (uint32_t)v);
    }
    return n_hot;
}
uint32_t debug_flags() {
    const char* f = debug_on() ? getenv("TGX_FLAGS") : nullptr;
    return f ? (uint32_t)atoi(f) : 0u;
}

uint32_t trace_blocks(const tgx_model* m, uint64_t n_samples) {
    return (uint32_t)std::max<uint64_t>(1, std::min<uint64_t>((n_samples + 3) / 4, (uint64_t)m->num_cus * 8));
}
int waves_for_units(int waves, uint64_t units, uint64_t n_blocks) {
    const uint64_t rows_wanted = (units + n_blocks - 1) / n_blocks;
    return (int)std::max<uint64_t>(1, std::min<uint64_t>((uint64_t)waves, (rows_wanted + 3) / 4));
}
uint32_t claim_chunk_for(uint64_t n_bytes, uint64_t units) {
    const uint64_t avg = units ? n_bytes / units : 0;
    return (uint32_t)std::min<uint64_t>(16, std::max<uint64_t>(1, 4096 / std::max<uint64_t>(1, avg)));
}

struct Stamps {
    unsigned long long* d = nullptr;
    size_t n_waves = 0;
};
Stamps stamps_begin(tgx_model* m, Pass& pass, char which, size_t n_waves) {
    const char* e = debug_on() ? getenv("TGX_STAMPS") : nullptr;
    Stamps st;
    st.n_waves = n_waves;
    if (!e || *e != which || pass.alloc(n_waves * 64, &st.d) != hipSuccess || hipMemsetAsync(st.d, 0, n_waves * 64, m->stream) != hipSuccess)
        st.d = nullptr;
    return st;
}
void stamps_report(tgx_model* m, const Stamps& st, int ppl, const char* what, const char* unit, std::initializer_list<const char*> phases) {
// ... 70 lines not shown
         (w2.empty() || hipMemcpyAsync(m->d_wvalues, w2.data(), ((size_t)nv + 1) * 8, hipMemcpyHostToDevice, m->stream) == hipSuccess) &&
         hipStreamSynchronize(m->stream) == hipSuccess;
    if (!ok) return fail(TGX_ERR_DEVICE, "value re-rank failed: %s", hipGetErrorString(hipGetLastError()));
    m->value_coverage = std::move(cov);
    hp.mark("re-rank");
    return pass.done();
}

tgx::EncodeParams base_encode_params(const tgx_model* m, const tgx_corpus* c, uint64_t seed) {
    tgx::EncodeParams p{};
    p.text = c->d_text;
    p.offs = c->d_offs;
    p.order = c->d_order;
    p.n_samples = c->n_samples;
    p.trie = m->d_trie;
    p.tokid = m->d_tokid;
    p.root_base = m->flat.table[0].base & ~tgx::kTerminalBit;
    p.lm = m->lm;
    p.n_slots = (uint32_t)m->flat.table.size();
    p.bp = c->d_bp;
    p.tmp = c->d_tmp;
    p.counts = c->d_counts;
    p.status = c->d_status;
    p.bp8 = reinterpret_cast<uint8_t*>(c->d_bp.get());
    p.tokhash = m->d_tokhash;
    p.tokhash_mask = m->tokhash.mask;
    p.tokhash_seed = m->tokhash.seed;
    p.err_sample = &m->d_ctrl->err;
    p.queue = &m->d_ctrl->queue;
    p.seed = seed;
    p.trace_carry = (c->n_samples && c->n_bytes / c->n_samples < 2048) ? 1u : 0u;
    p.trace_stride = tgx::kTraceStride;
    return p;
}

tgx_status redo_long_matches(tgx_model* m, tgx_corpus* c, const tgx::EncodeParams& p) {
    unsigned long long n_redo = 0;
    HIP_TRY(hipMemcpyAsync(&n_redo, &m->d_ctrl->encode_redo, 8, hipMemcpyDeviceToHost, m->stream));
    HIP_TRY(hipStreamSynchronize(m->stream));
    if (n_redo > c->n_samples) return fail(TGX_ERR_DEVICE, "redo list longer than the batch");
    m->last_redo_samples = n_redo;
    if (n_redo) {
        tgx::EncodeParams q = p;
        q.order = c->d_counts;
        q.n_samples = n_redo;
        HIP_TRY(hipMemsetAsync(&m->d_ctrl->queue, 0x00, 8, m->stream));
        time_begin(m, "encode2_kernel");
        HIP_TRY(tgx::launch_encode2(q, (uint32_t)m->num_cus, true, m->stream));
        time_end(m);
    }
    return TGX_OK;
}

tgx_status run_encode_kernel(tgx_model* m, tgx_corpus* c, double dropout, uint64_t seed, Pass& pass) {
    tgx_status st = ensure_scratch(c);
    if (st != TGX_OK) return st;
    HIP_TRY(hipMemsetAsync(&m->d_ctrl->queue, 0x00, 8, m->stream));
    HIP_TRY(hipMemsetAsync(&m->d_ctrl->err, 0xFF, 8, m->stream));
    tgx::EncodeParams p = base_encode_params(m, c, seed);
    p.dropout = dropout;
    if (const char* e = knob("TGX_TRACE_CARRY")) p.trace_carry = atoi(e) ? 1u : 0u;
    if (const char* e = knob("TGX_TRACE_STRIDE")) p.trace_stride = (uint32_t)std::min(3, std::max(0, atoi(e)));
    p.flags = debug_flags();
    const char* force = knob("TGX_PATH");
    const bool use4 = m->lm <= 16 && m->scores_finite && m->d_tokhash && !(force && strcmp(force, "fused") == 0);
    const bool use2 = !use4 && m->lm <= 32 && m->scores_finite && m->d_tokhash && !(force && strcmp(force, "fused") == 0);
    const bool long_tokens = m->lm > 16;
    const bool use5 = (use4 || use2) && m->have_trie8 &&
                      !(force && (strcmp(force, "rows4") == 0 || strcmp(force, "rows2") == 0 || strcmp(force, "rows4l") == 0));
    if (debug_on())
        fprintf(stderr, "[tgx] encode: S=%llu N=%llu lm=%u path=%s slots=%zu root_base=%u values=%u\n",
                (unsigned long long)c->n_samples, (unsigned long long)c->n_bytes, p.lm, use4 ? (use5 ? "rows5" : "rows4") : (use2 ? "rows2" : "fused"),
                m->flat.table.size(), p.root_base, m->n_values);
    m->last_lean_items = 0;
    if (use5) {
        {
            const tgx_status rst = ensure_value_ranks(m, c);
            if (rst != TGX_OK) return rst;
        }
        m->last_redo_samples = 0;
        int e6_bpc = 2;
        if (const char* e = knob("TGX_E6_BPC")) e6_bpc = std::min(4, std::max(1, atoi(e)));
        uint32_t n_hot6 = std::min(m->n_values, tgx::encode6_max_hot(160u * 1024u / (uint32_t)e6_bpc, 0u));
        uint32_t pool6 = 0;
        bool e6_usable = true;
        if (n_hot6 < m->n_values) {
            pool6 = 128;
            if (const char* e = knob("TGX_E6_POOL")) pool6 = (uint32_t)std::min(192, std::max(0, atoi(e)));
            if ((uint64_t)m->n_values + tgx::encode6_pool_total(pool6) > 65535ull) {
                pool6 = 0;
                e6_usable = knob("TGX_E6_POOL") != nullptr || knob("TGX_LONG_THRESHOLD") != nullptr;
            }
            n_hot6 = std::min(m->n_values, tgx::encode6_max_hot(160u * 1024u / (uint32_t)e6_bpc, pool6));
        }
        n_hot6 = knob_cap_hot("TGX_E5_HOT", n_hot6);
        const bool cold6 = n_hot6 < m->n_values;
        uint64_t n_long = 0;
        uint32_t corun_cus = 0;
        if (c->n_samples && !long_tokens && e6_usable) {
            const auto count_ge = [&](uint64_t thr) {
                return (uint64_t)(std::partition_point(c->h_sorted_len.begin(), c->h_sorted_len.end(),
                                                       [thr](uint32_t len) { return len >= thr; }) - c->h_sorted_len.begin());
            };
            if (const char* e = knob("TGX_LONG_THRESHOLD")) {
                const uint64_t thr = (uint64_t)std::max(0ll, atoll(e));
                if (thr) n_long = count_ge(thr);
            } else {
                const double N = (double)c->n_bytes;
                const double c5 = m->n_values > tgx::encode5_max_hot(false, 8, 4, 160u * 1024u) ? 0.135e-6 : 0.108e-6;
                auto cost = [&](uint64_t k) {
                    const double bytes_long = k ? (double)c->h_sorted_cum[k - 1] : 0.0;
                    const double t6 = k ? std::max((double)c->h_sorted_len[0] * (cold6 ? 0.042e-6 : 0.0369e-6), bytes_long / (cold6 ? 46e9 : 55e9)) + 20e-6 : 0.0;
                    const double rest_max = k < c->n_samples ? (double)c->h_sorted_len[k] : 0.0;
                    const double t5 = std::max(rest_max * c5, (N - bytes_long) / 88e9);
                    return t6 + t5;
                };
                double best = cost(0);
                for (uint64_t thr = 1024; thr <= c->max_len; thr *= 2) {
                    const uint64_t k = count_ge(thr);
                    const double ck = cost(k);
                    if (k && ck < best * 0.9) {
                        best = ck;
                        n_long = k;
                    }
                }
                const double c6 = cold6 ? 0.042e-6 : 0.0369e-6, r6 = (cold6 ? 46e9 : 55e9) / (double)m->num_cus;
                double best_co = best * 0.9;
                uint64_t k_co = 0;
                static const uint64_t thrs[] = {8192, 12288, 16384, 24576, 32768, 40960, 49152};
                static const uint32_t shares[] = {32, 48, 64, 96, 128, 160, 192};
                const bool corun_off = (knob("TGX_CORUN") && atoi(knob("TGX_CORUN")) == 0) || m->corun_wait_timeouts != 0 ||
                                       m->n_values > tgx::encode5_max_hot(false, 8, 4, 160u * 1024u);
                for (uint64_t thr : thrs) {
                    if (corun_off || thr > c->max_len || e6_bpc != 2) break;
                    const uint64_t k = count_ge(thr);
                    if (!k || k >= c->n_samples) continue;
                    const double bytes_long = (double)c->h_sorted_cum[k - 1];
                    const double r_max = (double)c->h_sorted_len[k], r_bytes = N - bytes_long;
                    for (uint32_t X : shares) {
                        if ((int)X >= m->num_cus) break;
                        const double t6 = std::max((double)c->h_sorted_len[0] * c6, bytes_long / (X * r6)) + 20e-6;
                        const double t5 = std::max(r_max * 0.12e-6, r_bytes / ((double)(m->num_cus - (int)X) / (double)m->num_cus * 70e9));
                        const double t = std::max(t5, t6);
                        if (t < best_co) {
                            best_co = t;
                            k_co = k;
                            corun_cus = X;
                        }
                    }
                }
                if (corun_cus) n_long = k_co;
            }
            if (const char* e = knob("TGX_CORUN")) {
                const int v = atoi(e);
                corun_cus = (v > 0 && v < m->num_cus && n_long > 0 && n_long < c->n_samples && e6_bpc == 2) ? (uint32_t)v : 0u;
            }
        }
        const int cus5 = m->num_cus - (int)corun_cus;
        const uint64_t rest_n = c->n_samples - n_long;
        const uint64_t rest_bytes = c->n_bytes - (n_long ? c->h_sorted_cum[n_long - 1] : 0);
        const uint64_t rest_max = rest_n ? c->h_sorted_len[n_long] : 0;
        int ppl = 4, bpc = 1, hot_waves = 16;
        int compact = kE5CompactDepth;
        if (const char* e = knob("TGX_E5_COMPACT")) compact = (strcmp(e, "off") == 0 || atoi(e) == 0) ? 0 : std::min(8, std::max(4, atoi(e)));
        bool lean = tgx::encode5_has_lean(dropout > 0.0, long_tokens);
        if (const char* e = knob("TGX_E5_LEAN")) lean = lean && atoi(e) != 0;
        const bool step_ok = m->lean_scores_ok;
        {
            int ps4 = 0;
            HIP_TRY(tgx::encode5_waves_per_simd(dropout > 0.0, false, 4, long_tokens, compact, lean, step_ok, &ps4));
            hot_waves = std::min(16, ps4 * 4);
            const int least = long_tokens ? 12 : 13;
            while (hot_waves >= least && m->n_values > tgx::encode5_max_hot(long_tokens, hot_waves, 4, 160u * 1024u)) hot_waves--;
            if (hot_waves < least) {
                hot_waves = 0;
                if (!long_tokens) {
                    if (m->n_values <= tgx::encode5_max_hot(false, 13, 3, 160u * 1024u)) {
                        ppl = 3;
                        hot_waves = 13;
                    } else if (m->n_values <= tgx::encode5_max_hot(false, 16, 2, 160u * 1024u)) {
                        ppl = 2;
                    } else {
                        ppl = 3;
                    }
                }
            }
        }
        int balance_waves = 0;
        if (rest_max > 0) {
            const uint64_t rows_bal = (rest_bytes + rest_max - 1) / rest_max;
            const uint64_t wb = (rows_bal + 4ull * (uint64_t)cus5 - 1) / (4ull * (uint64_t)cus5);
            if (wb <= 10) {
                balance_waves = (int)std::max<uint64_t>(4, wb);
                ppl = 4;
                hot_waves = 0;
            }
        }
        if (const char* e = long_tokens ? nullptr : knob("TGX_PPL")) {
            const int v = atoi(e);
            if (v >= 1 && v <= 4) {
                ppl = v;
                bpc = ppl >= 3 ? 1 : 2;
            }
        }
        knob_int("TGX_BPC", 1, 8, &bpc);
        const uint32_t budget = 160u * 1024u / (uint32_t)bpc;
        bool cold = false;
        int per_simd = 0;
        HIP_TRY(tgx::encode5_waves_per_simd(dropout > 0.0, false, ppl, long_tokens, compact, lean, step_ok, &per_simd));
        int waves = std::min(16, (per_simd / bpc) * 4);
        if ((ppl == 4 || ppl == 3) && bpc == 1 && hot_waves > 0) waves = std::min(waves, hot_waves);
        if (m->n_values > tgx::encode5_max_hot(long_tokens, waves, ppl, budget)) {
            cold = true;
            HIP_TRY(tgx::encode5_waves_per_simd(dropout > 0.0, true, ppl, long_tokens, compact, lean, step_ok, &per_simd));
            waves = std::min(16, (per_simd / bpc) * 4);
        }
        if (balance_waves > 0 && ppl == 4 && bpc == 1) waves = std::min(waves, balance_waves);
        waves = waves_for_units(waves, rest_n, (uint64_t)cus5 * bpc);
        knob_int("TGX_WAVES", 1, 16, &waves);
        while (waves > 1 && tgx::encode5_max_hot(long_tokens, waves, ppl, budget) < 16u) waves--;
        uint32_t n_hot = std::min(m->n_values, tgx::encode5_max_hot(long_tokens, waves, ppl, budget));
        n_hot = knob_cap_hot("TGX_E5_HOT", n_hot);
        cold = n_hot < m->n_values;
        m->last_n_hot = n_hot;
        m->last_lean_items = !lean ? 0u : ((rest_n ? (uint32_t)tgx::encode5_lean_items(cold, ppl, step_ok) : 0u) |
                                           (n_long ? (uint32_t)tgx::encode6_lean_items() << 8 : 0u));
        m->last_encode_waves_per_cu = std::min(bpc, per_simd / ((waves + 3) / 4)) * waves;
        const uint64_t rows_per_block = 4 * (uint64_t)waves;
        const uint32_t blocks5 = (uint32_t)std::max<uint64_t>(
            1, std::min<uint64_t>((rest_n + rows_per_block - 1) / rows_per_block, (uint64_t)cus5 * bpc));
        tgx::Encode5Params q{};
        q.trie8 = m->d_trie8;
        q.trie_bytes = (uint32_t)(m->flat.table.size() * sizeof(tgx::Trie8Rec));
        q.values = m->d_values;
        q.root_base = m->root_base8;
        q.n_values = m->n_values;
        q.n_hot = n_hot;
        q.claim_chunk = claim_chunk_for(c->n_bytes, c->n_samples);
        if (const char* e = knob("TGX_CLAIM_CHUNK")) q.claim_chunk = (uint32_t)std::min(64, std::max(1, atoi(e)));
        m->last_long_samples = n_long;
        m->last_corun_cus = n_long ? corun_cus : 0u;
        tgx::EncodeParams p6 = p;
        tgx::Encode5Params q6 = q;
        uint32_t blocks6 = 0;
        if (n_long) {
            p6.n_samples = n_long;
            blocks6 = (uint32_t)std::min<uint64_t>((n_long + 3) / 4, (uint64_t)(corun_cus ? (int)corun_cus : m->num_cus) * (uint64_t)e6_bpc);
            q6.n_hot = n_hot6;
            q6.pool = cold6 ? pool6 : 0u;
            if (!corun_cus) {
                time_begin(m, "encode6_kernel");
                HIP_TRY(tgx::launch_encode6(p6, q6, cold6, lean, blocks6, m->stream));
                time_end(m);
                HIP_TRY(hipMemsetAsync(&m->d_ctrl->queue, 0x00, 8, m->stream));
            } else {
                if (!m->stream2) {
                    HIP_TRY(hipStreamCreateWithFlags(&m->stream2, hipStreamNonBlocking));
                    HIP_TRY(hipEventCreateWithFlags(&m->ev_fork, hipEventDisableTiming));
                    HIP_TRY(hipEventCreateWithFlags(&m->ev_join, hipEventDisableTiming));
                    HIP_TRY(hipHostMalloc((void**)&m->h_started, 64, hipHostMallocMapped | hipHostMallocPortable));
                }
                *reinterpret_cast<volatile unsigned int*>(m->h_started) = 0u;
                q.started = m->h_started;
                p6.queue = &m->d_ctrl->queue6;
                HIP_TRY(hipMemsetAsync(&m->d_ctrl->queue6, 0x00, 8, m->stream));
                HIP_TRY(hipEventRecord(m->ev_fork, m->stream));
                HIP_TRY(hipStreamWaitEvent(m->stream2, m->ev_fork, 0));
            }
            p.order = c->d_order + n_long;
            p.n_samples = c->n_samples - n_long;
        }
        const Stamps stamps5 = stamps_begin(m, pass, '1', (size_t)blocks5 * (size_t)waves);
        p.stamps = stamps5.d;
        time_begin(m, "encode5_kernel");
        {
            if (long_tokens) {
                p.redo_count = &m->d_ctrl->encode_redo;
                p.redo_list = c->d_counts;
                HIP_TRY(hipMemsetAsync(&m->d_ctrl->encode_redo, 0x00, 8, m->stream));
            }
            const hipError_t le = tgx::launch_encode5(p, q, cold, ppl, long_tokens, compact, lean, step_ok, waves, blocks5, corun_cus && n_long ? 84u * 1024u : 0u, m->stream);
            if (le != hipSuccess) return fail(TGX_ERR_DEVICE, "encode5 launch failed: %s", hipGetErrorString(le));
        }
        bool joined = false, joined_slot = false;
        if (n_long && corun_cus) {
            const bool slot = m->n_timed + 1 < kMaxTimed;
            if (slot) {
                KernelTime& tb = m->timed[m->n_timed + 1];
                tb.name = "encode6_kernel";
                tb.used = true;
                (void)hipEventRecord(tb.start, m->stream2);
            }
            {
                const auto t0 = std::chrono::steady_clock::now();
                volatile unsigned int* started = m->h_started;
                bool timed_out = false;
                while (*started < blocks5 && !(timed_out = std::chrono::steady_clock::now() - t0 >= std::chrono::milliseconds(2))) {
                }
                if (timed_out && *started < blocks5) m->corun_wait_timeouts++;
            }
            const hipError_t l6 = tgx::launch_encode6(p6, q6, cold6, lean, blocks6, m->stream2);
            if (slot) (void)hipEventRecord(m->timed[m->n_timed + 1].stop, m->stream2);
            (void)hipEventRecord(m->ev_join, m->stream2);
            if (l6 != hipSuccess) return fail(TGX_ERR_DEVICE, "encode6 launch failed: %s", hipGetErrorString(l6));
            joined = true;
            joined_slot = slot;
        }
        time_end(m);
        if (joined) {
            if (joined_slot) m->n_timed++;
            HIP_TRY(hipStreamWaitEvent(m->stream, m->ev_join, 0));
        }
        if (stamps5.d) stamps_report(m, stamps5, ppl, "encode5 stamps", "iteration", {"switch", "text+reset", "walk", "relax", "store"});
        p.stamps = nullptr;
        if (long_tokens) {
            const tgx_status rst = redo_long_matches(m, c, p);
            if (rst != TGX_OK) return rst;
        }
        p.order = c->d_order;
        p.n_samples = c->n_samples;
        const uint32_t blocks_t = trace_blocks(m, c->n_samples);
        Stamps stamps_t;
        if (!long_tokens) stamps_t = stamps_begin(m, pass, '2', (size_t)blocks_t * 4);
        p.stamps = stamps_t.d;
        time_begin(m, long_tokens ? "trace32_kernel" : "trace_kernel");
        if (long_tokens) HIP_TRY(tgx::launch_trace32(p, blocks_t, true, m->stream));
        else HIP_TRY(tgx::launch_trace(p, blocks_t, m->stream));
        time_end(m);
        if (stamps_t.d) stamps_report(m, stamps_t, 0, "trace stamps", "window", {"setup", "loads", "hops", "append+lookups", "-"});
        p.stamps = nullptr;
    } else if (use4) {
        int ppl = 1, waves = 10, bpc = 2;
        const double gbps4[3] = {60.0, 50.0, 34.0}, chain4_ms[3] = {13.5, 10.7, 9.1};
        auto cost4 = [&](double bytes, double longest, int* ppl_out) {
            double best_t = 0;
            int best_ppl = 1;
            for (int i = 0; i < 3; i++) {
                const double t = std::max(bytes / (gbps4[i] * 1e9), longest / 65536.0 * chain4_ms[i] * 1e-3);
                if (i == 0 || t < best_t * 0.95) {
                    best_t = t;
                    best_ppl = 1 << i;
                }
            }
            if (ppl_out) *ppl_out = best_ppl;
            return best_t;
        };
        m->last_long_samples = 0;
        m->last_redo_samples = 0;
        cost4((double)c->n_bytes, c->n_samples ? (double)c->h_sorted_len[0] : 0.0, &ppl);
        if (const char* e = knob("TGX_PPL")) {
            const int v = atoi(e);
            if (v == 1 || v == 2 || v == 4) ppl = v;
        }
        if (ppl == 2) { waves = 5; bpc = 2; }
        if (ppl == 4) { waves = 5; bpc = 1; }
        knob_int("TGX_WAVES", 1, 16, &waves);
        knob_int("TGX_BPC", 1, 8, &bpc);
        bool root = ppl == 1;
        if (const char* e = knob("TGX_ROOT")) root = root && atoi(e) != 0;
        while (waves > 1 && tgx::encode4_lds_bytes(waves, ppl, root) > (160u * 1024u) / (uint32_t)bpc) waves--;
        {
            int per_simd = 0;
            HIP_TRY(tgx::encode4_waves_per_simd(dropout > 0.0, ppl, root, &per_simd));
            if (bpc * ((waves + 3) / 4) > per_simd && ppl == 1) {
                waves = 4;
                bpc = std::min(5, per_simd);
                root = false;
                HIP_TRY(tgx::encode4_waves_per_simd(dropout > 0.0, ppl, root, &per_simd));
            }
            m->last_encode_waves_per_cu = std::min(bpc * ((waves + 3) / 4), per_simd) * 4 >= bpc * waves
                                              ? bpc * waves
                                              : per_simd / ((waves + 3) / 4) * waves;
        }
        const uint64_t rows_per_block = 4 * (uint64_t)waves;
        const uint32_t blocks4 = (uint32_t)std::max<uint64_t>(
            1, std::min<uint64_t>((p.n_samples + rows_per_block - 1) / rows_per_block, (uint64_t)m->num_cus * bpc));
        Stamps stamps4;
        if (dropout <= 0.0 && ppl == 1) stamps4 = stamps_begin(m, pass, '1', (size_t)blocks4 * (size_t)waves);
        p.stamps = stamps4.d;
        time_begin(m, "encode4_kernel");
        HIP_TRY(tgx::launch_encode4(p, ppl, waves, blocks4, root, m->stream));
        time_end(m);
        if (stamps4.d) stamps_report(m, stamps4, 0, "stamps", "iteration", {"switch", "text", "walk", "relax", "store"});
        p.stamps = nullptr;
        p.order = c->d_order;
        p.n_samples = c->n_samples;
        time_begin(m, "trace_kernel");
        HIP_TRY(tgx::launch_trace(p, trace_blocks(m, c->n_samples), m->stream));
        time_end(m);
    } else if (use2) {
        const bool rows2 = force && strcmp(force, "rows2") == 0;
        m->last_redo_samples = 0;
        if (!rows2) {
            p.redo_count = &m->d_ctrl->encode_redo;
            p.redo_list = c->d_counts;
            HIP_TRY(hipMemsetAsync(&m->d_ctrl->encode_redo, 0x00, 8, m->stream));
            time_begin(m, "encode4l_kernel");
            HIP_TRY(tgx::launch_encode4l(p, (uint32_t)m->num_cus, m->stream));
            time_end(m);
            const tgx_status rst = redo_long_matches(m, c, p);
            if (rst != TGX_OK) return rst;
        } else {
            time_begin(m, "encode2_kernel");
            HIP_TRY(tgx::launch_encode2(p, (uint32_t)m->num_cus, false, m->stream));
            time_end(m);
        }
        time_begin(m, "trace32_kernel");
        HIP_TRY(tgx::launch_trace32(p, trace_blocks(m, c->n_samples), !rows2, m->stream));
        time_end(m);
    } else {
        time_begin(m, "encode_kernel");
        HIP_TRY(tgx::launch_encode(p, grid_blocks(m, c->n_samples), m->stream));
        time_end(m);
    }
    return TGX_OK;
}

tgx_status check_no_path(tgx_model* m, const tgx_corpus* c) {
    unsigned long long bad = m->h_ctrl->err;
    if (bad == ~0ULL) return TGX_OK;
    if (bad & (1ULL << 62))
        return fail(TGX_ERR_DEVICE, "internal error: corrupt back-pointer (sample or text byte %llu)",
                    (unsigned long long)(bad & ~(1ULL << 62)));
    uint64_t n = c->h_offs[bad + 1] - c->h_offs[bad];
    set_error_detail(bad, n, n);
    return fail(TGX_ERR_NO_PATH, "no path to position %llu/%llu", (unsigned long long)n,
                (unsigned long long)n);
}

tgx_status compact_ids(tgx_model* m, tgx_corpus* c, tgx_result* r, const char* what) {
    const uint64_t S = c->n_samples;
    if (!c->d_scan_tmp) {
        if (tgx::scan_temp_bytes(S, &c->scan_tmp_bytes) != hipSuccess) return fail(TGX_ERR_DEVICE, "scan temp-size query failed");
        if (c->scan_tmp_bytes && c->d_scan_tmp.alloc(m->device, c->scan_tmp_bytes) != hipSuccess)
            return fail(TGX_ERR_DEVICE, "out of device memory (scan)");
    }
    time_begin(m, "scan_counts_kernel");
    if (tgx::launch_scan(c->d_counts, r->d_offs, S, c->d_scan_tmp, c->scan_tmp_bytes, m->stream) != hipSuccess)
        return fail(TGX_ERR_DEVICE, "scan launch failed");
    time_end(m);
    if (hipMemcpyAsync(&m->h_ctrl->err, &m->d_ctrl->err, 8, hipMemcpyDeviceToHost, m->stream) != hipSuccess ||
        hipMemcpyAsync(&m->h_ctrl->total_tokens, r->d_offs + S, 8, hipMemcpyDeviceToHost, m->stream) != hipSuccess ||
        hipStreamSynchronize(m->stream) != hipSuccess)
        return fail(TGX_ERR_DEVICE, "%s pass failed: %s", what, hipGetErrorString(hipGetLastError()));
    const tgx_status st = check_no_path(m, c);
    if (st != TGX_OK) return st;
    r->n_tokens = m->h_ctrl->total_tokens;
    if (r->d_ids.alloc(m->device, (size_t)r->n_tokens * 4 + 256) != hipSuccess)
        return fail(TGX_ERR_DEVICE, "out of device memory (result ids)");
    tgx::CompactParams cp{};
    cp.offs = c->d_offs;
    cp.order = c->d_order;
    cp.n_samples = S;
    cp.tmp = c->d_tmp;
    cp.out_offs = r->d_offs;
    cp.ids = r->d_ids;
    const bool rows = S && r->n_tokens / S < 128;
    const uint64_t units = rows ? 16 : 4;
    const uint32_t blocks = (uint32_t)std::max<uint64_t>(1, std::min<uint64_t>((S + units - 1) / units, (uint64_t)m->num_cus * 8));
    time_begin(m, "compact_kernel");
    if (tgx::launch_compact(cp, blocks, rows, m->stream) != hipSuccess) return fail(TGX_ERR_DEVICE, "compact launch failed");
    time_end(m);
    return TGX_OK;
}

template <class Run>
tgx_status on_uploaded_batch(const tgx_model* m, const uint8_t* text, const uint64_t* offs, uint64_t n_samples, Run run) {
    tgx_corpus* c = nullptr;
    tgx_status st = tgx_corpus_upload(m->device, text, offs, n_samples, &c);
    if (st != TGX_OK) return st;
    st = run(c);
    tgx_corpus_free(c);
    return st;
}

}

const char* tgx_last_error(void) { return g_err_msg.c_str(); }

void tgx_last_error_detail(uint64_t* sample, uint64_t* pos, uint64_t* len) {
    if (sample) *sample = g_err_sample;
    if (pos) *pos = g_err_pos;
    if (len) *len = g_err_len;
}

int tgx_abi_version(void) { return TGX_ABI_VERSION; }
int tgx_device_count(void) { return usable_device_count(); }
void tgx_free(void* p) { free(p); }
void tgx_pool_trim(int device) { pool_trim(device); }
void* tgx_host_alloc(uint64_t bytes) {
    if (require_device() != TGX_OK) return nullptr;
    void* p = nullptr;
    if (hipHostMalloc(&p, bytes ? (size_t)bytes : 1, hipHostMallocPortable) != hipSuccess) {
        (void)hipGetLastError();
        fail(TGX_ERR_DEVICE, "out of page-locked host memory (%llu bytes)", (unsigned long long)bytes);
        return nullptr;
    }
    return p;
}
void tgx_host_free(void* p) {
    if (p) (void)hipHostFree(p);
}
// ... 432 lines not shown
    const uint64_t* ho = c->h_offs.data();
    std::stable_sort(order.begin(), order.end(), [ho](uint32_t a, uint32_t b) {
        return ho[a + 1] - ho[a] > ho[b + 1] - ho[b];
    });

    c->max_len = n_samples ? ho[order[0] + 1] - ho[order[0]] : 0;
    c->h_sorted_len.resize(n_samples);
    c->h_sorted_cum.resize(n_samples);
    for (uint64_t i = 0, run = 0; i < n_samples; i++) {
        c->h_sorted_len[i] = (uint32_t)(ho[order[i] + 1] - ho[order[i]]);
        run += c->h_sorted_len[i];
        c->h_sorted_cum[i] = run;
    }
    HIP_TRY(hipSetDevice(device));
    HIP_TRY(c->d_text_alloc.alloc(device, (size_t)c->n_bytes + 512));
    c->d_text = c->d_text_alloc + 256;
    HIP_TRY(hipMemset(c->d_text_alloc, 0, 256));
    HIP_TRY(c->d_offs.alloc(device, (size_t)(n_samples + 1) * 8));
    HIP_TRY(c->d_order.alloc(device, (size_t)n_samples * 4 + 4));
    if (c->n_bytes && from != TextFrom::Caller)
        HIP_TRY(copy_sync(c->d_text, text + base, c->n_bytes, from == TextFrom::Device ? hipMemcpyDeviceToDevice : hipMemcpyHostToDevice, device));
    HIP_TRY(hipMemset(c->d_text + c->n_bytes, 0, 256));
    HIP_TRY(hipMemcpy(c->d_offs, c->h_offs.data(), (n_samples + 1) * 8, hipMemcpyHostToDevice));
    if (n_samples) HIP_TRY(hipMemcpy(c->d_order, order.data(), n_samples * 4, hipMemcpyHostToDevice));
    *out = c.release();
    return TGX_OK;
}

tgx_status tgx_corpus_upload(int device, const uint8_t* text, const uint64_t* offs,
                             uint64_t n_samples, tgx_corpus** out) {
    return corpus_create("tgx_corpus_upload", device, text, TextFrom::Host, offs, n_samples, out);
}

void tgx_corpus_free(tgx_corpus* c) { delete c; }

uint64_t tgx_corpus_num_samples(const tgx_corpus* c) { return c ? c->n_samples : 0; }
uint64_t tgx_corpus_num_bytes(const tgx_corpus* c) { return c ? c->n_bytes : 0; }


static tgx_status encode_corpus_locked(tgx_model* m, tgx_corpus* c, double dropout, uint64_t seed,
                                       tgx_result** out) {
    HIP_TRY(hipSetDevice(m->device));
    {
        const tgx_status est = ensure_encode_tables(m);
        if (est != TGX_OK) return est;
    }
    m->n_timed = 0;
    const uint64_t S = c->n_samples;

    Pass pass(m);
    tgx_result* r = pass.new_result(S);
    if (r->d_offs.alloc(m->device, (size_t)(S + 1) * 8) != hipSuccess)
        return fail(TGX_ERR_DEVICE, "out of device memory (result offsets)");
    tgx_status st = run_encode_kernel(m, c, dropout, seed, pass);
    if (st != TGX_OK) return st;
    st = compact_ids(m, c, r, "encode");
    if (st != TGX_OK) return st;
    if (hipStreamSynchronize(m->stream) != hipSuccess)
        return fail(TGX_ERR_DEVICE, "compact failed: %s", hipGetErrorString(hipGetLastError()));
    m->last_alg_bytes = c->n_bytes + 4 * r->n_tokens + 16 * (S + 1);
    *out = pass.release_result();
    return pass.done();
}

tgx_status tgx_encode_corpus(tgx_model* m, tgx_corpus* c, double dropout, uint64_t seed,
                             tgx_result** out) {
    if (!m || !c || !out) return fail(TGX_ERR_INVALID, "tgx_encode_corpus: NULL argument");
    *out = nullptr;
    if (m->device != c->device) return fail(TGX_ERR_INVALID, "model and corpus on different devices");
    std::lock_guard<std::mutex> lk(m->mu);
    std::lock_guard<std::mutex> lkc(c->mu);
    return encode_corpus_locked(m, c, dropout, seed, out);
}

tgx_status tgx_encode_batch(tgx_model* m, const uint8_t* text, const uint64_t* offs,
                            uint64_t n_samples, double dropout, uint64_t seed, tgx_result** out) {
    if (!m || !out) return fail(TGX_ERR_INVALID, "tgx_encode_batch: NULL argument");
    *out = nullptr;
    return on_uploaded_batch(m, text, offs, n_samples, [&](tgx_corpus* c) { return tgx_encode_corpus(m, c, dropout, seed, out); });
}

tgx_status tgx_encode_batch_host(tgx_model* m, const uint8_t* text, const uint64_t* offs, uint64_t n_samples, double dropout,
                                 uint64_t seed, uint32_t* ids_out, uint64_t ids_cap, uint64_t* offs_out, uint64_t* n_tokens) {
    if (!m || !offs_out || !n_tokens || (n_samples && !offs)) return fail(TGX_ERR_INVALID, "tgx_encode_batch_host: NULL argument");
    *n_tokens = 0;
    offs_out[0] = 0;
    if (n_samples == 0) return TGX_OK;
    for (uint64_t i = 0; i < n_samples; i++)
        if (offs[i + 1] < offs[i]) return fail(TGX_ERR_INVALID, "offsets not monotone at %llu", (unsigned long long)i);
    const uint64_t N = offs[n_samples] - offs[0];
    std::vector<uint64_t> cut(1, 0);
    {
        uint64_t chunk = 256ull << 20;
        if (dropout > 0.0) chunk = ~0ull;
        if (const char* e = knob("TGX_E2E_CHUNK_MB")) {
            const long v = atol(e);
            if (v > 0 && dropout <= 0.0) chunk = (uint64_t)v << 20;
        }
        uint64_t start = offs[0];
        for (uint64_t i = 0; i < n_samples; i++)
            if (offs[i + 1] - start >= chunk && i + 1 < n_samples) {
                cut.push_back(i + 1);
                start = offs[i + 1];
            }
        cut.push_back(n_samples);
    }
    const size_t C = cut.size() - 1;
    struct ChunkState {
        tgx_corpus* corpus = nullptr;
        tgx_result* result = nullptr;
        uint64_t tokens = 0;
        int stage = 0;
// ... 2884 lines not shown
    return pass.done();
}

tgx_status tgx_encode_corpus_nbest(tgx_model* m, tgx_corpus* c, uint32_t nbest, double* scores, uint32_t* n_found, tgx_result** out) {
    if (const tgx_status dst = require_device()) return dst;
    if (!m || !c || !out) return fail(TGX_ERR_INVALID, "tgx_encode_corpus_nbest: NULL argument");
    *out = nullptr;
    if (m->device != c->device) return fail(TGX_ERR_INVALID, "model and corpus on different devices");
    std::lock_guard<std::mutex> lk(m->mu);
    const tgx_status st = nbest_check(m, nbest);
    if (st != TGX_OK) return st;
    std::lock_guard<std::mutex> lkc(c->mu);
    return nbest_corpus_locked(m, c, nbest, scores, n_found, out);
}

tgx_status tgx_encode_batch_nbest(tgx_model* m, const uint8_t* text, const uint64_t* offs, uint64_t n_samples, uint32_t nbest,
                                  double* scores, uint32_t* n_found, tgx_result** out) {
    if (const tgx_status dst = require_device()) return dst;
    if (!m || !out) return fail(TGX_ERR_INVALID, "tgx_encode_batch_nbest: NULL argument");
    *out = nullptr;
    {
        std::lock_guard<std::mutex> lk(m->mu);
        const tgx_status st = nbest_check(m, nbest);
        if (st != TGX_OK) return st;
    }
    return on_uploaded_batch(m, text, offs, n_samples, [&](tgx_corpus* c) { return tgx_encode_corpus_nbest(m, c, nbest, scores, n_found, out); });
}


int tgx_last_kernel_times(const tgx_model* m, const char** names, float* ms, int cap) {
    if (!m) return 0;
    int n = 0;
    for (int i = 0; i < m->n_timed && n < cap; i++) {
        float t = 0.f;
        if (hipEventElapsedTime(&t, m->timed[i].start, m->timed[i].stop) != hipSuccess) t = -1.f;
        if (names) names[n] = m->timed[i].name;
        if (ms) ms[n] = t;
        n++;
    }
    return n;
}

uint32_t tgx_last_encode_waves_per_cu(const tgx_model* m) { return m ? (uint32_t)m->last_encode_waves_per_cu : 0u; }
uint64_t tgx_last_algorithmic_bytes(const tgx_model* m) { return m ? m->last_alg_bytes : 0; }
uint64_t tgx_last_encode_redo_samples(const tgx_model* m) { return m ? m->last_redo_samples : 0; }
uint64_t tgx_last_encode_long_samples(const tgx_model* m) { return m ? m->last_long_samples : 0; }
uint64_t tgx_last_estep_pieces(const tgx_model* m) { return m ? m->last_estep_pieces : 0; }
uint64_t tgx_last_estep_redo(const tgx_model* m) { return m ? m->last_estep_redo : 0; }
uint32_t tgx_last_encode_corun_cus(const tgx_model* m) { return m ? m->last_corun_cus : 0; }
uint32_t tgx_encode_corun_timeouts(const tgx_model* m) { return m ? m->corun_wait_timeouts : 0; }
uint32_t tgx_model_score_values(const tgx_model* m) { return m && m->have_trie8 ? m->n_values : 0u; }
uint32_t tgx_last_encode_hot_values(const tgx_model* m) { return m ? m->last_n_hot : 0u; }
uint32_t tgx_last_encode_lean_items(const tgx_model* m) { return m ? m->last_lean_items : 0u; }
```

tokengeex_amd/csrc/trace_body.h:

```cpp
#pragma once
#include <hip/hip_runtime.h>
#include <stdint.h>

#include "device_common.h"
#include "kernels.h"

namespace tgx {

constexpr uint32_t kTraceRing = 128;

#define TGX_TRACE_STAMP(i)                                             \
    if (STAMP) {                                                       \
        __builtin_amdgcn_sched_barrier(0);                             \
        const uint64_t _now = (uint64_t)__builtin_amdgcn_s_memtime(); \
        __builtin_amdgcn_s_waitcnt(0xC07F);                            \
        __builtin_amdgcn_sched_barrier(0);                             \
        seg[i] += _now - t_last;                                       \
        t_last = _now;                                                 \
    }

__device__ __forceinline__ int32_t trace_lane_addr(int32_t p) {
    return (p < 0 ? 0 : p) << 2;
}
__device__ __forceinline__ int32_t trace_square(int32_t p) {
    const int32_t got = __builtin_amdgcn_ds_bpermute(trace_lane_addr(p), p);
    return p < 0 ? p : got;
}
template <int K>
__device__ __forceinline__ uint64_t trace_hops(uint32_t prev, int32_t& qq) {
    static_assert(K >= 0 && K <= 3, "strides of 1, 2, 4, 8 tokens");
    if constexpr (K == 0) {
        uint64_t ends = 0;
        while (qq >= 0) {
            asm("s_bitset1_b64 %0, %1" : "+s"(ends) : "s"(qq));
            qq = (int32_t)readlane_u32(prev, (uint32_t)qq);
        }
        return ends;
    } else {
        int32_t p[K + 1];
        p[0] = (int32_t)prev;
#pragma unroll
        for (int k = 1; k <= K; ++k) p[k] = trace_square(p[k - 1]);
        uint64_t visited = 0;
        while (qq >= 0) {
            asm("s_bitset1_b64 %0, %1" : "+s"(visited) : "s"(qq));
            qq = (int32_t)readlane_u32((uint32_t)p[K], (uint32_t)qq);
        }
        uint64_t on = visited;
#pragma unroll
        for (int k = K - 1; k >= 0; --k) {
            const bool send = __builtin_amdgcn_inverse_ballot_w64(on) && p[k] >= 0;
            const int32_t got = __builtin_amdgcn_ds_permute(send ? trace_lane_addr(p[k]) : 63 << 2, 1);
            on |= __builtin_amdgcn_ballot_w64(got != 0) & ~(1ULL << 63);
        }
        return on;
    }
}

template <bool CARRY> struct TraceRingEntry { using type = uint2; };
template <> struct TraceRingEntry<true> { using type = uint4; };
template <uint32_t LM, bool PERM, bool STAMP, bool CARRY, int K>
__device__ __forceinline__ void trace_body(const EncodeParams& P, typename TraceRingEntry<CARRY>::type* ring) {
    static_assert(LM == 16 || LM == 32, "token lengths of up to 16 or 32 bytes");
    constexpr uint32_t LMASK = LM - 1u;
    constexpr int NW = (int)LM / 4;
    const uint32_t lane = threadIdx.x & 63u;
    const uint32_t wpb = blockDim.x >> 6;
    const uint32_t n_waves = gridDim.x * wpb;
    const uint32_t wave_id = (uint32_t)__builtin_amdgcn_readfirstlane((int)(blockIdx.x * wpb + (threadIdx.x >> 6)));
    const uint4* __restrict__ table = reinterpret_cast<const uint4*>(P.tokhash);
    uint64_t seg[6] = {0, 0, 0, 0, 0, 0};
    uint64_t t_last = STAMP ? (uint64_t)__builtin_amdgcn_s_memtime() : 0;
    uint32_t iters = 0;
    const uint64_t n_rounds = (P.n_samples + n_waves - 1) / n_waves;
    constexpr uint32_t kNone = 0xFFFFFFFFu;
    auto sample_of_round = [&](uint64_t rnd) -> uint32_t {
        const uint64_t k = rnd * n_waves + ((rnd & 1u) ? (uint64_t)(n_waves - 1u - wave_id) : (uint64_t)wave_id);
        return (rnd < n_rounds && k < P.n_samples) ? P.order[k] : kNone;
    };
    struct MetaRaw {
        uint64_t beg, end;
        uint32_t reach;
    };
    struct Meta {
        uint32_t s;
        uint64_t beg;
        uint32_t n, reach_n;
    };
    auto meta_request = [&](uint32_t smp) -> MetaRaw {
        MetaRaw r{0, 0, 1u};
        if (smp != kNone) {
            r.beg = P.offs[smp];
            r.end = P.offs[smp + 1];
            r.reach = P.status[smp];
        }
        return r;
    };
    auto meta_read = [&](uint32_t smp, const MetaRaw& r) -> Meta {
        Meta mt{smp, 0, 0, 1u};
        if (smp != kNone) {
            mt.beg = first_u64(r.beg);
            mt.n = (uint32_t)(first_u64(r.end) - mt.beg);
            mt.reach_n = (mt.n == 0) ? 1u : (uint32_t)__builtin_amdgcn_readfirstlane((int)r.reach);
        }
        return mt;
    };
    auto first_window = [&](const Meta& mt) -> uint32_t {
        if (mt.s == kNone || mt.n == 0 || !mt.reach_n || (P.flags & 4u)) return 0u;
        const uint8_t* __restrict__ bpn = P.bp8 + bp8_base(mt.beg, mt.s);
        const uint32_t wq0 = (mt.n - 1u) & ~63u;
        return (wq0 + lane < mt.n) ? (uint32_t)bpn[PERM ? bp8_perm(wq0 + lane) : wq0 + lane] : 0u;
    };
    uint32_t head = 0, fill = 0;
    uint64_t flush_beg = 0, flush_out_top = 0;
    auto lookup = [&](uint32_t m) {
        if (lane < m && !(P.flags & 16u)) {
            const auto e = ring[(head + lane) & (kTraceRing - 1u)];
            uint32_t len;
            uint64_t end, out;
            if constexpr (CARRY) {
                len = e.y >> 16;
                end = ((uint64_t)(e.y & 0xFFFFu) << 32) | e.x;
                out = ((uint64_t)e.w << 32) | e.z;
            } else {
                len = e.y;
                end = flush_beg + e.x;
                out = flush_out_top - 1u - lane;
            }
            struct __attribute__((packed, aligned(1))) Bytes16 { uint32_t w[4]; };
            const Bytes16* __restrict__ src = reinterpret_cast<const Bytes16*>(P.text + (end - len));
            uint32_t b[8] = {0, 0, 0, 0, 0, 0, 0, 0};
#pragma unroll
            for (int j = 0; j < NW; j += 4) {
                const Bytes16 raw = src[j / 4];
#pragma unroll
                for (int i = 0; i < 4; ++i) {
                    const uint32_t nb = len > 4u * (j + i) ? len - 4u * (j + i) : 0u;
                    b[j + i] = nb >= 4u ? raw.w[i] : (raw.w[i] & ((1u << (8u * nb)) - 1u));
                }
            }
            const uint64_t hk = LM == 16 ? tok_hash64_dev(b[0], b[1], b[2], b[3], len, P.tokhash_seed)
                                         : tok_hash64_long_dev(b, len, P.tokhash_seed);
            uint32_t slot = (uint32_t)hk & P.tokhash_mask;
            uint32_t id = 0;
            bool found = false;
            for (uint32_t probe = 0; probe <= P.tokhash_mask && !found; ++probe) {
                const uint4 t = load_rec(table, slot);
                if (t.w == 0u) break;
                if (t.x == (uint32_t)hk && t.y == (uint32_t)(hk >> 32)) {
                    id = t.z;
                    found = true;
                }
                slot = (slot + 1u) & P.tokhash_mask;
            }
            if (!found) atomicMin(P.err_sample, (unsigned long long)((end - len) & ((1ULL << 62) - 1ULL)) | (1ULL << 62));
            P.tmp[out] = id;
        }
        if constexpr (!CARRY) flush_out_top -= m;
        head = (head + m) & (kTraceRing - 1u);
        fill -= m;
    };
    Meta cur;
    {
        const uint32_t s0 = (uint32_t)__builtin_amdgcn_readfirstlane((int)sample_of_round(0));
        cur = meta_read(s0, meta_request(s0));
    }
    uint32_t s_next_raw = sample_of_round(1);
    uint32_t h_first = first_window(cur);
    for (uint64_t rnd = 0; rnd < n_rounds; ++rnd) {
        const uint32_t s_next = (uint32_t)__builtin_amdgcn_readfirstlane((int)s_next_raw);
        const uint32_t s_after_raw = sample_of_round(rnd + 2);
        const MetaRaw nxt_raw = meta_request(s_next);
        const uint32_t s = cur.s;
        const uint64_t beg = cur.beg;
        const uint32_t n = cur.n;
        const uint32_t reach_n = cur.reach_n;
        const bool have = s != kNone;
        const uint8_t* __restrict__ bp = P.bp8 + (have ? bp8_base(beg, s) : 0);
        uint32_t total = 0;
        uint64_t out_top = beg + n;
        flush_beg = beg;
        flush_out_top = out_top;
        int64_t q = (have && reach_n) ? (int64_t)n - 1 : (int64_t)-1;
        if (P.flags & 4u) q = -1;

        uint32_t h_cur = h_first;
        TGX_TRACE_STAMP(0)
        while (q >= 0) {
            iters++;
            const uint32_t wq = (uint32_t)q & ~63u;
            const uint32_t idx = wq + lane;
            const uint32_t h = h_cur;
            uint32_t prev = lane - ((h & LMASK) + 1u);
            asm volatile("" : "+v"(prev) : : "memory");
            uint32_t h_next = 0;
            if (wq >= 64u) h_next = (uint32_t)bp[PERM ? bp8_perm(wq - 64u + lane) : wq - 64u + lane];
            TGX_TRACE_STAMP(1)
            int32_t qq = (int32_t)((uint32_t)q - wq);
            const uint64_t ends = trace_hops<K>(prev, qq);
            q = (int64_t)wq + qq;
            const uint32_t cnt = (uint32_t)__popcll(ends);
            TGX_TRACE_STAMP(2)
            if ((ends >> lane) & 1ULL) {
                const uint32_t below = __builtin_amdgcn_mbcnt_hi((uint32_t)(ends >> 32), __builtin_amdgcn_mbcnt_lo((uint32_t)ends, 0u));
                if constexpr (CARRY) {
                    const uint64_t end = beg + idx + 1u, out = out_top - 1u - (cnt - 1u - below);
                    ring[(head + fill + (cnt - 1u - below)) & (kTraceRing - 1u)] =
                        make_uint4((uint32_t)end, (uint32_t)(end >> 32) | (((h & LMASK) + 1u) << 16), (uint32_t)out, (uint32_t)(out >> 32));
                } else {
                    ring[(head + fill + (cnt - 1u - below)) & (kTraceRing - 1u)] = make_uint2(idx + 1u, (h & LMASK) + 1u);
                }
            }
            fill += cnt;
            total += cnt;
            out_top -= cnt;
            __builtin_amdgcn_wave_barrier();
            if (fill >= 64u) lookup(64u);
            TGX_TRACE_STAMP(3)
            h_cur = h_next;
        }
        const Meta nxt = meta_read(s_next, nxt_raw);
        h_first = first_window(nxt);
        if constexpr (!CARRY) {
            if (fill) lookup(fill);
        }
        if (have && lane == 0) {
            P.counts[s] = total;
            if (!reach_n) atomicMin(P.err_sample, (unsigned long long)s);
        }
        cur = nxt;
        s_next_raw = s_after_raw;
    }
    if (fill) lookup(fill);
    if (STAMP && lane == 0 && P.stamps) {
        unsigned long long* o = P.stamps + (size_t)wave_id * 8u;
        for (int i = 0; i < 5; ++i) o[i] = seg[i];
        o[5] = iters;
    }
}

}
```

Measured before the change: 71710.

## Count tokens in the forward pass and write ids in place during trace

The encode5 forward kernel now carries a running token count in the upper bits of the backpointer word, so per-sample token counts are known before the trace. The offsets are scanned first, and the trace kernel then writes ids straight to their final positions. This removes the temporary id buffer and the separate compaction pass. It adds a DPP read and a select to each relax step in the hot DP loop, plus a count-mismatch check in the trace.

```diff
diff --git a/include/tgx.h b/include/tgx.h
--- a/include/tgx.h
+++ b/include/tgx.h
@@ -305,6 +305,7 @@
 uint32_t tgx_model_score_values(const tgx_model *m);
 uint32_t tgx_last_encode_hot_values(const tgx_model *m);
 uint32_t tgx_last_encode_lean_items(const tgx_model *m);
+int tgx_last_encode_ids_in_place(const tgx_model *m);
 
 static inline double tgx_dropout_u01(uint64_t seed, uint64_t sample, uint64_t pos, uint32_t len) {
     uint64_t x = seed ^ (sample * 0x9E3779B97F4A7C15ULL) ^ (pos * 0xC2B2AE3D27D4EB4FULL) ^
diff --git a/tokengeex_amd/_lib.py b/tokengeex_amd/_lib.py
--- a/tokengeex_amd/_lib.py
+++ b/tokengeex_amd/_lib.py
@@ -91,6 +91,7 @@
     "tgx_model_score_values": (_u32, [_vp]),
     "tgx_last_encode_hot_values": (_u32, [_vp]),
     "tgx_last_encode_lean_items": (_u32, [_vp]),
+    "tgx_last_encode_ids_in_place": (_i, [_vp]),
     "tgx_last_encode_long_samples": (_u64, [_vp]),
     "tgx_last_estep_pieces": (_u64, [_vp]),
     "tgx_last_estep_redo": (_u64, [_vp]),
@@ -1239,6 +1240,9 @@
     def last_encode_lean_step(self) -> bool:
         return bool(self.last_encode_lean_items()[0] & 1)
 
+    def last_encode_ids_in_place(self) -> bool:
+        return bool(lib.tgx_last_encode_ids_in_place(self._h))
+
     def last_encode_long_samples(self) -> int:
         return lib.tgx_last_encode_long_samples(self._h)
 
diff --git a/tokengeex_amd/build.py b/tokengeex_amd/build.py
--- a/tokengeex_amd/build.py
+++ b/tokengeex_amd/build.py
@@ -9,7 +9,7 @@
 CSRC = os.path.join(HERE, "csrc")
 OUT = os.path.join(HERE, "libtgx.so")
 SOURCES = ["kernels.hip", "estep.hip", "encode2.hip", "encode4l.hip", "encode5.hip", "estep4.hip", "estep4l.hip", "estep7.hip", "cuts.hip", "pairs.hip", "generate.hip", "sample.hip", "nbest.hip", "layout.hip", "assemble.hip", "fim.hip", "decode.hip", "spans.hip", "front.hip", "norm.hip", "tgx_api.cpp", "host_twins.cpp", "trie_build.cpp", "prune_host.cpp", "frontback.cpp", "unicode_norm.cpp"]
-HEADERS = ["api_internal.h", "kernels.h", "sample.h", "nbest.h", "layout.h", "assemble.h", "fim.h", "decode.h", "spans.h", "front.h", "norm.h", "device_common.h", "lean_gate.h", "trace_body.h", "trie_build.h", "unicode_tables.h", os.path.join("..", "..", "include", "tgx.h")]
+HEADERS = ["api_internal.h", "kernels.h", "sample.h", "nbest.h", "layout.h", "assemble.h", "fim.h", "decode.h", "spans.h", "front.h", "norm.h", "device_common.h", "lean_gate.h", "ids_in_place.h", "trace_body.h", "trie_build.h", "unicode_tables.h", os.path.join("..", "..", "include", "tgx.h")]
 ARCH = "gfx950"
 
 
diff --git a/tokengeex_amd/csrc/device_common.h b/tokengeex_amd/csrc/device_common.h
--- a/tokengeex_amd/csrc/device_common.h
+++ b/tokengeex_amd/csrc/device_common.h
@@ -174,7 +174,15 @@
 template <int LN>
 __device__ __forceinline__ bool relax5_reached(uint32_t fhi) { return (LN & kLeanStep) ? fhi < kLeanUnreachedHi : fhi != 0xFFF00000u; }
 
-template <int U, int LN = 0>
+template <int U>
+__device__ __forceinline__ uint32_t relax5_count_cand(uint32_t bpv) {
+    uint32_t ff = 0xFFu;
+    asm("" : "+v"(ff));
+    const uint32_t from = (uint32_t)__builtin_amdgcn_update_dpp(0, (int)bpv, 0x150 + U, 0xF, 0xF, false);
+    return (from | ff) + (1u + (uint32_t)U);
+}
+
+template <int U, int LN = 0, bool CNT = false>
 __device__ __forceinline__ void relax5_step(double sv, double& acc, uint32_t& bpv, uint32_t& fin, uint32_t& fhi) {
     constexpr uint64_t MU = kRowLane0 << U;
     double best;
@@ -186,10 +194,11 @@
     const double cand = best + sv;
     const uint64_t take = __builtin_amdgcn_fcmp(cand, acc_r, 2 );
     asm("v_max_f64 %0, %1, %2" : "=v"(acc) : "v"(acc_r), "v"(cand));
-    bpv = sel_imm_u32<U>(take, bpv);
-}
-
-template <int U, int LN>
+    if constexpr (CNT) bpv = sel_u32(take, relax5_count_cand<U>(bpv), bpv);
+    else bpv = sel_imm_u32<U>(take, bpv);
+}
+
+template <int U, int LN, bool CNT = false>
 __device__ __forceinline__ void relax5_lean_step(double sv, double& acc, uint32_t& bpv, uint32_t& fin) {
     constexpr uint64_t MU = kRowLane0 << U;
     double best;
@@ -202,7 +211,8 @@
     const double cand = best + sv;
     const uint64_t take = __builtin_amdgcn_fcmp(cand, acc_r, 2 );
     asm("v_max_f64 %0, %1, %2" : "=v"(acc) : "v"(acc_r), "v"(cand));
-    bpv = sel_imm_u32<U>(take, bpv);
+    if constexpr (CNT) bpv = sel_u32(take, relax5_count_cand<U>(bpv), bpv);
+    else bpv = sel_imm_u32<U>(take, bpv);
 }
 
 
diff --git a/tokengeex_amd/csrc/encode5.hip b/tokengeex_amd/csrc/encode5.hip
--- a/tokengeex_amd/csrc/encode5.hip
+++ b/tokengeex_amd/csrc/encode5.hip
@@ -299,10 +299,10 @@
         t_last = _now;                                                 \
     }
 
-template <bool DROPOUT, bool COLD, int PPL, bool LONG, int CK = 0, int LN = 0>
+template <bool DROPOUT, bool COLD, int PPL, bool LONG, int CK = 0, int LN = 0, bool CNT = false>
 __global__ __launch_bounds__(1024, (PPL == 1 ? 8 : (PPL == 2 ? 6 : (PPL == 3 ? 4 : 1)))) void encode5_kernel(EncodeParams P, Encode5Params Q) {
     static_assert(!LONG || PPL == 4, "the long-token build runs four positions per lane");
-    static_assert(LN == 0 || (!LONG && !DROPOUT), "the long-token and dropout builds keep the kernel as it was");
+    static_assert((LN == 0 && !CNT) || (!LONG && !DROPOUT), "the long-token and dropout builds keep the kernel as it was");
     extern __shared__ __align__(16) unsigned char smem[];
     constexpr uint32_t LM = LONG ? 32 : 16;
     constexpr uint32_t SPAN = 16u * PPL;
@@ -529,7 +529,7 @@
                     }
                     continue;
                 }
-                if constexpr (LN == 0) {
+                if constexpr (LN == 0 && !CNT) {
                     if (COLD) {
                         double sv[8], sw[8];
                         e5_scores_cold<8>(lds0, cold_values, cw, 0, hot_bytes, sv);
@@ -578,8 +578,8 @@
                 } else {
                     const bool full = !(LN & kLeanStep) || ((end_groups >> g) & 1u) != 0u;
 #define E5_STEP(U, SV)                                                   \
-        if (FULL) relax5_step<U, LN>(SV, acc, bpv, fin[g], fhi);              \
-        else relax5_lean_step<U, LN>(SV, acc, bpv, fin[g]);
+        if (FULL) relax5_step<U, LN, CNT>(SV, acc, bpv, fin[g], fhi);         \
+        else relax5_lean_step<U, LN, CNT>(SV, acc, bpv, fin[g]);
                     auto steps = [&](auto full_tag) {
                         constexpr bool FULL = decltype(full_tag)::value;
                         if (COLD) {
@@ -654,7 +654,10 @@
             if (left < SPAN) {
 #pragma unroll
                 for (int g = 0; g < PPL; ++g)
-                    if (left == 16u * g + l) P.status[s] = (n == 0u || reached[g]) ? 1u : 0u;
+                    if (left == 16u * g + l) {
+                        P.status[s] = (n == 0u || reached[g]) ? 1u : 0u;
+                        if constexpr (CNT) P.counts[s] = (n != 0u && reached[g]) ? fin[g] >> 8 : 0u;
+                    }
                 need_new = true;
             } else {
                 p0 += SPAN;
@@ -1179,7 +1182,19 @@
     return step_ok ? items : lean_without_step(items);
 }
 int encode6_lean_items() { return kE6Lean; }
-static encode5_fn pick_encode5(bool dropout, bool cold, int ppl, bool long_tokens, int compact, bool lean, bool step_ok) {
+#ifdef TGX_E5_CNT
+constexpr bool kE5CntHot = TGX_E5_CNT != 0, kE5CntHot2 = TGX_E5_CNT != 0, kE5CntCold = TGX_E5_CNT != 0, kE5CntCold3 = TGX_E5_CNT != 0;
+#else
+constexpr bool kE5CntHot = true;
+constexpr bool kE5CntHot2 = true;
+constexpr bool kE5CntCold = true;
+constexpr bool kE5CntCold3 = true;
+#endif
+bool encode5_counts(bool dropout, bool cold, int ppl, bool long_tokens) {
+    if (dropout || long_tokens) return false;
+    return cold ? (ppl == 3 ? kE5CntCold3 : kE5CntCold) : (ppl == 2 ? kE5CntHot2 : kE5CntHot);
+}
+static encode5_fn pick_encode5(bool dropout, bool cold, int ppl, bool long_tokens, int compact, bool lean, bool step_ok, bool count) {
     if (long_tokens) {
         if (cold) return dropout ? encode5_kernel<true, true, 4, true> : encode5_kernel<false, true, 4, true>;
         return dropout ? encode5_kernel<true, false, 4, true> : encode5_kernel<false, false, 4, true>;
@@ -1196,28 +1211,34 @@
         if (ppl == 3) return encode5_kernel<true, false, 3, false>;
         return encode5_kernel<true, false, 4, false>;
     }
-#define TGX_E5K(C, PL, LN) \
-    (compact == 4 ? encode5_kernel<false, C, PL, false, 4, LN> : compact == 5 ? encode5_kernel<false, C, PL, false, 5, LN> \
-     : compact == 6 ? encode5_kernel<false, C, PL, false, 6, LN> : compact == 7 ? encode5_kernel<false, C, PL, false, 7, LN> \
-     : compact == 8 ? encode5_kernel<false, C, PL, false, 8, LN> : encode5_kernel<false, C, PL, false, 0, LN>)
-#define TGX_E5L(LNH, LNC, LNC3) \
+#define TGX_E5K(C, PL, LN, CN) \
+    (compact == 4 ? encode5_kernel<false, C, PL, false, 4, LN, CN> : compact == 5 ? encode5_kernel<false, C, PL, false, 5, LN, CN> \
+     : compact == 6 ? encode5_kernel<false, C, PL, false, 6, LN, CN> : compact == 7 ? encode5_kernel<false, C, PL, false, 7, LN, CN> \
+     : compact == 8 ? encode5_kernel<false, C, PL, false, 8, LN, CN> : encode5_kernel<false, C, PL, false, 0, LN, CN>)
+#define TGX_E5L(LNH, LNC, LNC3, CN) \
     if (cold) { \
-        if (ppl == 1) return encode5_kernel<false, true, 1, false, 0, LNC>; \
-        if (ppl == 2) return TGX_E5K(true, 2, LNC); \
-        if (ppl == 3) return TGX_E5K(true, 3, LNC3); \
-        return TGX_E5K(true, 4, LNC); \
+        if (ppl == 1) return encode5_kernel<false, true, 1, false, 0, LNC, CN && kE5CntCold>; \
+        if (ppl == 2) return TGX_E5K(true, 2, LNC, CN && kE5CntCold); \
+        if (ppl == 3) return TGX_E5K(true, 3, LNC3, CN && kE5CntCold3); \
+        return TGX_E5K(true, 4, LNC, CN && kE5CntCold); \
     } \
-    if (ppl == 1) return encode5_kernel<false, false, 1, false, 0, LNH>; \
-    if (ppl == 2) return TGX_E5K(false, 2, LNH); \
-    if (ppl == 3) return TGX_E5K(false, 3, LNH); \
-    return TGX_E5K(false, 4, LNH);
-    if (lean && step_ok) {
-        TGX_E5L(kE5LeanHot, kE5LeanCold, kE5LeanCold3)
-    }
-    if (lean) {
-        TGX_E5L(lean_without_step(kE5LeanHot), lean_without_step(kE5LeanCold), lean_without_step(kE5LeanCold3))
-    }
-    TGX_E5L(0, 0, 0)
+    if (ppl == 1) return encode5_kernel<false, false, 1, false, 0, LNH, CN && kE5CntHot>; \
+    if (ppl == 2) return TGX_E5K(false, 2, LNH, CN && kE5CntHot2); \
+    if (ppl == 3) return TGX_E5K(false, 3, LNH, CN && kE5CntHot); \
+    return TGX_E5K(false, 4, LNH, CN && kE5CntHot);
+#define TGX_E5C(CN) \
+    if (lean && step_ok) { \
+        TGX_E5L(kE5LeanHot, kE5LeanCold, kE5LeanCold3, CN) \
+    } \
+    if (lean) {   \
+        TGX_E5L(lean_without_step(kE5LeanHot), lean_without_step(kE5LeanCold), lean_without_step(kE5LeanCold3), CN) \
+    } \
+    TGX_E5L(0, 0, 0, CN)
+    if (count) {
+        TGX_E5C(true)
+    }
+    TGX_E5C(false)
+#undef TGX_E5C
 #undef TGX_E5L
 #undef TGX_E5K
 }
@@ -1237,9 +1258,10 @@
     return budget > fixed + 64u ? (budget - fixed) / 8u : 0u;
 }
 
-hipError_t encode5_waves_per_simd(bool dropout, bool cold, int ppl, bool long_tokens, int compact, bool lean, bool step_ok, int* out) {
+hipError_t encode5_waves_per_simd(bool dropout, bool cold, int ppl, bool long_tokens, int compact, bool lean, bool step_ok, bool count, int* out) {
     hipFuncAttributes attr;
-    hipError_t e = hipFuncGetAttributes(&attr, reinterpret_cast<const void*>(pick_encode5(dropout, cold, ppl, long_tokens, compact, lean && encode5_has_lean(dropout, long_tokens), step_ok)));
+    hipError_t e = hipFuncGetAttributes(&attr, reinterpret_cast<const void*>(pick_encode5(dropout, cold, ppl, long_tokens, compact, lean && encode5_has_lean(dropout, long_tokens), step_ok,
+                                                                                             count && encode5_counts(dropout, cold, ppl, long_tokens))));
     if (e != hipSuccess) return e;
     const int regs = (attr.numRegs + 7) & ~7;
     *out = regs > 0 ? (512 / regs > 8 ? 8 : 512 / regs) : 8;
@@ -1285,14 +1307,15 @@
     return hipGetLastError();
 }
 
-hipError_t launch_encode5(const EncodeParams& p, Encode5Params q, bool cold, int ppl, bool long_tokens, int compact, bool lean, bool step_ok,
+hipError_t launch_encode5(const EncodeParams& p, Encode5Params q, bool cold, int ppl, bool long_tokens, int compact, bool lean, bool step_ok, bool count,
                           int waves, uint32_t blocks, uint32_t min_lds, hipStream_t stream) {
     uint32_t lds = encode5_lds_layout(q.n_hot, long_tokens, waves, ppl, &q.list_off, &q.root_off, &q.idx_off);
     if (lds > 160u * 1024u || q.n_hot > q.n_values || (!cold && q.n_hot != q.n_values) || (long_tokens && ppl != 4) ||
         (compact != 0 && (compact < 4 || compact > 8)))
         return hipErrorInvalidValue;
     lean = lean && encode5_has_lean(p.dropout > 0.0, long_tokens);
-    encode5_fn fn = pick_encode5(p.dropout > 0.0, cold, ppl, long_tokens, compact, lean, step_ok);
+    if (count && !encode5_counts(p.dropout > 0.0, cold, ppl, long_tokens)) return hipErrorInvalidValue;
+    encode5_fn fn = pick_encode5(p.dropout > 0.0, cold, ppl, long_tokens, compact, lean, step_ok, count);
     hipError_t e = hipFuncSetAttribute(reinterpret_cast<const void*>(fn), hipFuncAttributeMaxDynamicSharedMemorySize, 160 * 1024);
     if (e != hipSuccess) return e;
     if (lean && (e = lean_lds_check(reinterpret_cast<const void*>(fn))) != hipSuccess) return e;
diff --git a/tokengeex_amd/csrc/ids_in_place.h b/tokengeex_amd/csrc/ids_in_place.h
--- /dev/null
+++ b/tokengeex_amd/csrc/ids_in_place.h
@@ -0,0 +1,28 @@
+#pragma once
+#include <stdint.h>
+
+namespace tgx {
+
+constexpr uint64_t kCountFieldSamples = 1ull << 24;
+
+struct IdsInPlaceQuery {
+    bool rows5;
+    bool long_tokens;
+    bool dropout;
+    uint64_t n_long;
+    bool build_counts;
+    uint64_t max_len;
+    bool switched_on;
+    bool diagnostics;
+};
+
+inline bool ids_in_place(const IdsInPlaceQuery& q) {
+    return q.rows5 && !q.long_tokens && !q.dropout && q.n_long == 0 && q.build_counts && q.max_len < kCountFieldSamples &&
+           q.switched_on && !q.diagnostics;
+}
+
+inline uint32_t count_step_word(uint32_t from, uint32_t u) { return (from | 0xFFu) + (1u + u); }
+inline uint32_t count_of_word(uint32_t word) { return word >> 8; }
+constexpr uint32_t kCountNoStep = 0xFFu;
+
+}
diff --git a/tokengeex_amd/csrc/kernels.h b/tokengeex_amd/csrc/kernels.h
--- a/tokengeex_amd/csrc/kernels.h
+++ b/tokengeex_amd/csrc/kernels.h
@@ -260,19 +260,27 @@
 hipError_t launch_encode4(const EncodeParams& p, int ppl, int waves, uint32_t blocks, bool root, hipStream_t stream);
 uint32_t encode4_lds_bytes(int waves, int ppl, bool root);
 hipError_t launch_trace(const EncodeParams& p, uint32_t blocks, hipStream_t stream);
+struct TraceInPlace {
+    const uint64_t* out_offs;
+    uint32_t* ids;
+};
+hipError_t launch_trace_in_place(const EncodeParams& p, const TraceInPlace& o, uint32_t blocks, hipStream_t stream);
+constexpr unsigned long long kErrCorruptBp = 1ULL << 62;
+constexpr unsigned long long kErrCountMismatch = 1ULL << 61;
 uint32_t encode5_lds_layout(uint32_t n_hot, bool long_tokens, int waves, int ppl, uint32_t* list_off, uint32_t* root_off, uint32_t* idx_off);
 uint32_t encode5_max_hot(bool long_tokens, int waves, int ppl, uint32_t budget);
 bool encode5_has_lean(bool dropout, bool long_tokens);
 int encode5_lean_items(bool cold, int ppl, bool step_ok);
 int encode6_lean_items();
-hipError_t encode5_waves_per_simd(bool dropout, bool cold, int ppl, bool long_tokens, int compact, bool lean, bool step_ok, int* out);
+bool encode5_counts(bool dropout, bool cold, int ppl, bool long_tokens);
+hipError_t encode5_waves_per_simd(bool dropout, bool cold, int ppl, bool long_tokens, int compact, bool lean, bool step_ok, bool count, int* out);
 uint32_t encode6_lds_layout(uint32_t n_hot, uint32_t pool, uint32_t* root_off, uint32_t* ctrl_off, uint32_t* ring_off);
 uint32_t encode6_max_hot(uint32_t budget, uint32_t pool);
 uint32_t encode6_pool_total(uint32_t pool);
 hipError_t estep5_waves_per_simd(bool dropout, bool cold, int ppl, int* out);
 hipError_t launch_estep5_fwd(const struct Estep4Params& p, Encode5Params q, bool cold, int ppl, int waves, uint32_t blocks, hipStream_t stream);
 hipError_t launch_encode6(const EncodeParams& p, Encode5Params q, bool cold, bool lean, uint32_t blocks, hipStream_t stream);
-hipError_t launch_encode5(const EncodeParams& p, Encode5Params q, bool cold, int ppl, bool long_tokens, int compact, bool lean, bool step_ok,
+hipError_t launch_encode5(const EncodeParams& p, Encode5Params q, bool cold, int ppl, bool long_tokens, int compact, bool lean, bool step_ok, bool count,
                           int waves, uint32_t blocks, uint32_t min_lds, hipStream_t stream);
 hipError_t launch_encode2(const EncodeParams& p, uint32_t num_cus, bool permuted, hipStream_t stream);
 hipError_t launch_trace32(const EncodeParams& p, uint32_t blocks, bool permuted, hipStream_t stream);
diff --git a/tokengeex_amd/csrc/kernels.hip b/tokengeex_amd/csrc/kernels.hip
--- a/tokengeex_amd/csrc/kernels.hip
+++ b/tokengeex_amd/csrc/kernels.hip
@@ -500,10 +500,11 @@
     }
 }
 
-template <bool STAMP, bool CARRY, int K>
-__global__ __launch_bounds__(256) void trace_kernel(EncodeParams P) {
+template <bool STAMP, bool CARRY, int K, bool INPLACE = false>
+__global__ __launch_bounds__(256, INPLACE ? 8 : 1) void trace_kernel(EncodeParams P, TraceInPlace O) {
+    static_assert(!(STAMP && INPLACE), "the stamped build writes through tmp");
     __shared__ typename TraceRingEntry<CARRY>::type ring_all[4][kTraceRing];
-    trace_body<16, true, STAMP, CARRY, K>(P, ring_all[threadIdx.x >> 6]);
+    trace_body<16, true, STAMP, CARRY, K, INPLACE>(P, ring_all[threadIdx.x >> 6], O);
 }
 
 __global__ __launch_bounds__(1024) void scan_counts_kernel(const uint32_t* __restrict__ counts,
@@ -642,10 +643,10 @@
 template <bool STAMP, bool CARRY>
 static void launch_trace_stride(const EncodeParams& p, uint32_t blocks, hipStream_t stream) {
     switch (p.trace_stride) {
-        case 1: hipLaunchKernelGGL((trace_kernel<STAMP, CARRY, 1>), dim3(blocks), dim3(256), 0, stream, p); break;
-        case 2: hipLaunchKernelGGL((trace_kernel<STAMP, CARRY, 2>), dim3(blocks), dim3(256), 0, stream, p); break;
-        case 3: hipLaunchKernelGGL((trace_kernel<STAMP, CARRY, 3>), dim3(blocks), dim3(256), 0, stream, p); break;
-        default: hipLaunchKernelGGL((trace_kernel<STAMP, CARRY, 0>), dim3(blocks), dim3(256), 0, stream, p); break;
+        case 1: hipLaunchKernelGGL((trace_kernel<STAMP, CARRY, 1>), dim3(blocks), dim3(256), 0, stream, p, TraceInPlace{nullptr, nullptr}); break;
+        case 2: hipLaunchKernelGGL((trace_kernel<STAMP, CARRY, 2>), dim3(blocks), dim3(256), 0, stream, p, TraceInPlace{nullptr, nullptr}); break;
+        case 3: hipLaunchKernelGGL((trace_kernel<STAMP, CARRY, 3>), dim3(blocks), dim3(256), 0, stream, p, TraceInPlace{nullptr, nullptr}); break;
+        default: hipLaunchKernelGGL((trace_kernel<STAMP, CARRY, 0>), dim3(blocks), dim3(256), 0, stream, p, TraceInPlace{nullptr, nullptr}); break;
     }
 }
 hipError_t launch_trace(const EncodeParams& p, uint32_t blocks, hipStream_t stream) {
@@ -658,6 +659,24 @@
     return hipGetLastError();
 }
 
+template <bool CARRY>
+static void launch_trace_in_place_stride(const EncodeParams& p, const TraceInPlace& o, uint32_t blocks, hipStream_t stream) {
+    switch (p.trace_stride) {
+        case 1: hipLaunchKernelGGL((trace_kernel<false, CARRY, 1, true>), dim3(blocks), dim3(256), 0, stream, p, o); break;
+        case 2: hipLaunchKernelGGL((trace_kernel<false, CARRY, 2, true>), dim3(blocks), dim3(256), 0, stream, p, o); break;
+        case 3: hipLaunchKernelGGL((trace_kernel<false, CARRY, 3, true>), dim3(blocks), dim3(256), 0, stream, p, o); break;
+        default: hipLaunchKernelGGL((trace_kernel<false, CARRY, 0, true>), dim3(blocks), dim3(256), 0, stream, p, o); break;
+    }
+}
+hipError_t launch_trace_in_place(const EncodeParams& p, const TraceInPlace& o, uint32_t blocks, hipStream_t stream) {
+    if (p.stamps || !o.out_offs || !o.ids) return hipErrorInvalidValue;
+    if (p.trace_carry)
+        launch_trace_in_place_stride<true>(p, o, blocks, stream);
+    else
+        launch_trace_in_place_stride<false>(p, o, blocks, stream);
+    return hipGetLastError();
+}
+
 struct WidenU32 {
     __host__ __device__ uint64_t operator()(uint32_t x) const { return (uint64_t)x; }
 };
diff --git a/tokengeex_amd/csrc/tgx_api.cpp b/tokengeex_amd/csrc/tgx_api.cpp
--- a/tokengeex_amd/csrc/tgx_api.cpp
+++ b/tokengeex_amd/csrc/tgx_api.cpp
@@ -25,6 +25,7 @@
 #include "front.h"
 #include "kernels.h"
 #include "layout.h"
+#include "ids_in_place.h"
 #include "lean_gate.h"
 #include "spans.h"
 #include "nbest.h"
@@ -262,6 +263,7 @@
     uint32_t n_values = 0, root_base8 = 0;
     uint32_t last_n_hot = 0;
     bool lean_scores_ok = false;
+    bool last_ids_in_place = false;
     uint32_t last_lean_items = 0;
     bool have_trie8 = false;
     bool encode_tables_ready = false;
@@ -424,12 +426,12 @@
     m->n_timed++;
 }
 
-tgx_status ensure_scratch(tgx_corpus* c) {
+tgx_status ensure_scratch(tgx_corpus* c, bool with_tmp = true) {
     HIP_TRY(hipSetDevice(c->device));
     if (!c->d_bp) HIP_TRY(c->d_bp.alloc(c->device, std::max((size_t)c->n_bytes * 4 + 256, (size_t)c->n_bytes + 128 * (size_t)c->n_samples + 512)));
     if (!c->d_counts) HIP_TRY(c->d_counts.alloc(c->device, (size_t)c->n_samples * 4 + 256));
     if (!c->d_status) HIP_TRY(c->d_status.alloc(c->device, (size_t)c->n_samples * 4 + 256));
-    if (!c->d_tmp) HIP_TRY(c->d_tmp.alloc(c->device, (size_t)c->n_bytes * 4 + 256));
+    if (with_tmp && !c->d_tmp) HIP_TRY(c->d_tmp.alloc(c->device, (size_t)c->n_bytes * 4 + 256));
     return TGX_OK;
 }
 
@@ -606,8 +608,12 @@
     return TGX_OK;
 }
 
-tgx_status run_encode_kernel(tgx_model* m, tgx_corpus* c, double dropout, uint64_t seed, Pass& pass) {
-    tgx_status st = ensure_scratch(c);
+tgx_status check_no_path(tgx_model* m, const tgx_corpus* c);
+tgx_status scan_ids_offsets(tgx_model* m, tgx_corpus* c, tgx_result* r, const char* what, bool with_err);
+
+tgx_status run_encode_kernel(tgx_model* m, tgx_corpus* c, double dropout, uint64_t seed, Pass& pass, tgx_result* r) {
+    m->last_ids_in_place = false;
+    tgx_status st = ensure_scratch(c, false);
     if (st != TGX_OK) return st;
     HIP_TRY(hipMemsetAsync(&m->d_ctrl->queue, 0x00, 8, m->stream));
     HIP_TRY(hipMemsetAsync(&m->d_ctrl->err, 0xFF, 8, m->stream));
@@ -627,6 +633,10 @@
                 (unsigned long long)c->n_samples, (unsigned long long)c->n_bytes, p.lm, use4 ? (use5 ? "rows5" : "rows4") : (use2 ? "rows2" : "fused"),
                 m->flat.table.size(), p.root_base, m->n_values);
     m->last_lean_items = 0;
+    if (!use5) {
+        if ((st = ensure_scratch(c, true)) != TGX_OK) return st;
+        p.tmp = c->d_tmp;
+    }
     if (use5) {
         {
             const tgx_status rst = ensure_value_ranks(m, c);
@@ -720,9 +730,19 @@
         bool lean = tgx::encode5_has_lean(dropout > 0.0, long_tokens);
         if (const char* e = knob("TGX_E5_LEAN")) lean = lean && atoi(e) != 0;
         const bool step_ok = m->lean_scores_ok;
+        tgx::IdsInPlaceQuery iq{};
+        iq.rows5 = true;
+        iq.long_tokens = long_tokens;
+        iq.dropout = dropout > 0.0;
+        iq.n_long = n_long;
+        iq.build_counts = true;
+        iq.max_len = c->max_len;
+        iq.switched_on = !(knob("TGX_IDS_IN_PLACE") && atoi(knob("TGX_IDS_IN_PLACE")) == 0);
+        iq.diagnostics = p.flags != 0u || (debug_on() && getenv("TGX_STAMPS") != nullptr);
+        const bool want_count = r != nullptr && tgx::ids_in_place(iq);
         {
             int ps4 = 0;
-            HIP_TRY(tgx::encode5_waves_per_simd(dropout > 0.0, false, 4, long_tokens, compact, lean, step_ok, &ps4));
+            HIP_TRY(tgx::encode5_waves_per_simd(dropout > 0.0, false, 4, long_tokens, compact, lean, step_ok, want_count, &ps4));
             hot_waves = std::min(16, ps4 * 4);
             const int least = long_tokens ? 12 : 13;
             while (hot_waves >= least && m->n_values > tgx::encode5_max_hot(long_tokens, hot_waves, 4, 160u * 1024u)) hot_waves--;
@@ -761,12 +781,12 @@
         const uint32_t budget = 160u * 1024u / (uint32_t)bpc;
         bool cold = false;
         int per_simd = 0;
-        HIP_TRY(tgx::encode5_waves_per_simd(dropout > 0.0, false, ppl, long_tokens, compact, lean, step_ok, &per_simd));
+        HIP_TRY(tgx::encode5_waves_per_simd(dropout > 0.0, false, ppl, long_tokens, compact, lean, step_ok, want_count, &per_simd));
         int waves = std::min(16, (per_simd / bpc) * 4);
         if ((ppl == 4 || ppl == 3) && bpc == 1 && hot_waves > 0) waves = std::min(waves, hot_waves);
         if (m->n_values > tgx::encode5_max_hot(long_tokens, waves, ppl, budget)) {
             cold = true;
-            HIP_TRY(tgx::encode5_waves_per_simd(dropout > 0.0, true, ppl, long_tokens, compact, lean, step_ok, &per_simd));
+            HIP_TRY(tgx::encode5_waves_per_simd(dropout > 0.0, true, ppl, long_tokens, compact, lean, step_ok, want_count, &per_simd));
             waves = std::min(16, (per_simd / bpc) * 4);
         }
         if (balance_waves > 0 && ppl == 4 && bpc == 1) waves = std::min(waves, balance_waves);
@@ -777,6 +797,12 @@
         n_hot = knob_cap_hot("TGX_E5_HOT", n_hot);
         cold = n_hot < m->n_values;
         m->last_n_hot = n_hot;
+        iq.build_counts = tgx::encode5_counts(dropout > 0.0, cold, ppl, long_tokens);
+        const bool in_place = want_count && tgx::ids_in_place(iq);
+        if (!in_place) {
+            if ((st = ensure_scratch(c, true)) != TGX_OK) return st;
+            p.tmp = c->d_tmp;
+        }
         m->last_lean_items = !lean ? 0u : ((rest_n ? (uint32_t)tgx::encode5_lean_items(cold, ppl, step_ok) : 0u) |
                                            (n_long ? (uint32_t)tgx::encode6_lean_items() << 8 : 0u));
         m->last_encode_waves_per_cu = std::min(bpc, per_simd / ((waves + 3) / 4)) * waves;
@@ -833,7 +859,7 @@
                 p.redo_list = c->d_counts;
                 HIP_TRY(hipMemsetAsync(&m->d_ctrl->encode_redo, 0x00, 8, m->stream));
             }
-            const hipError_t le = tgx::launch_encode5(p, q, cold, ppl, long_tokens, compact, lean, step_ok, waves, blocks5, corun_cus && n_long ? 84u * 1024u : 0u, m->stream);
+            const hipError_t le = tgx::launch_encode5(p, q, cold, ppl, long_tokens, compact, lean, step_ok, in_place, waves, blocks5, corun_cus && n_long ? 84u * 1024u : 0u, m->stream);
             if (le != hipSuccess) return fail(TGX_ERR_DEVICE, "encode5 launch failed: %s", hipGetErrorString(le));
         }
         bool joined = false, joined_slot = false;
@@ -874,6 +900,14 @@
         p.order = c->d_order;
         p.n_samples = c->n_samples;
         const uint32_t blocks_t = trace_blocks(m, c->n_samples);
+        if (in_place) {
+            if ((st = scan_ids_offsets(m, c, r, "encode", false)) != TGX_OK) return st;
+            time_begin(m, "trace_kernel");
+            HIP_TRY(tgx::launch_trace_in_place(p, tgx::TraceInPlace{r->d_offs, r->d_ids}, blocks_t, m->stream));
+            time_end(m);
+            m->last_ids_in_place = true;
+            return TGX_OK;
+        }
         Stamps stamps_t;
         if (!long_tokens) stamps_t = stamps_begin(m, pass, '2', (size_t)blocks_t * 4);
         p.stamps = stamps_t.d;
@@ -973,16 +1007,19 @@
 tgx_status check_no_path(tgx_model* m, const tgx_corpus* c) {
     unsigned long long bad = m->h_ctrl->err;
     if (bad == ~0ULL) return TGX_OK;
-    if (bad & (1ULL << 62))
+    if (bad & tgx::kErrCorruptBp)
         return fail(TGX_ERR_DEVICE, "internal error: corrupt back-pointer (sample or text byte %llu)",
-                    (unsigned long long)(bad & ~(1ULL << 62)));
+                    (unsigned long long)(bad & ~tgx::kErrCorruptBp));
+    if (bad & tgx::kErrCountMismatch)
+        return fail(TGX_ERR_DEVICE, "internal error: the token count of sample %llu differs between the relaxation and the trace",
+                    (unsigned long long)(bad & ~tgx::kErrCountMismatch));
     uint64_t n = c->h_offs[bad + 1] - c->h_offs[bad];
     set_error_detail(bad, n, n);
     return fail(TGX_ERR_NO_PATH, "no path to position %llu/%llu", (unsigned long long)n,
                 (unsigned long long)n);
 }
 
-tgx_status compact_ids(tgx_model* m, tgx_corpus* c, tgx_result* r, const char* what) {
+tgx_status scan_ids_offsets(tgx_model* m, tgx_corpus* c, tgx_result* r, const char* what, bool with_err) {
     const uint64_t S = c->n_samples;
     if (!c->d_scan_tmp) {
         if (tgx::scan_temp_bytes(S, &c->scan_tmp_bytes) != hipSuccess) return fail(TGX_ERR_DEVICE, "scan temp-size query failed");
@@ -993,15 +1030,25 @@
     if (tgx::launch_scan(c->d_counts, r->d_offs, S, c->d_scan_tmp, c->scan_tmp_bytes, m->stream) != hipSuccess)
         return fail(TGX_ERR_DEVICE, "scan launch failed");
     time_end(m);
-    if (hipMemcpyAsync(&m->h_ctrl->err, &m->d_ctrl->err, 8, hipMemcpyDeviceToHost, m->stream) != hipSuccess ||
+    if ((with_err && hipMemcpyAsync(&m->h_ctrl->err, &m->d_ctrl->err, 8, hipMemcpyDeviceToHost, m->stream) != hipSuccess) ||
         hipMemcpyAsync(&m->h_ctrl->total_tokens, r->d_offs + S, 8, hipMemcpyDeviceToHost, m->stream) != hipSuccess ||
         hipStreamSynchronize(m->stream) != hipSuccess)
         return fail(TGX_ERR_DEVICE, "%s pass failed: %s", what, hipGetErrorString(hipGetLastError()));
-    const tgx_status st = check_no_path(m, c);
-    if (st != TGX_OK) return st;
+    if (with_err) {
+        const tgx_status st = check_no_path(m, c);
+        if (st != TGX_OK) return st;
+    }
     r->n_tokens = m->h_ctrl->total_tokens;
+    if (r->n_tokens > c->n_bytes) return fail(TGX_ERR_DEVICE, "internal error: %s pass counted more tokens than bytes", what);
     if (r->d_ids.alloc(m->device, (size_t)r->n_tokens * 4 + 256) != hipSuccess)
         return fail(TGX_ERR_DEVICE, "out of device memory (result ids)");
+    return TGX_OK;
+}
+
+tgx_status compact_ids(tgx_model* m, tgx_corpus* c, tgx_result* r, const char* what) {
+    const uint64_t S = c->n_samples;
+    const tgx_status sst = scan_ids_offsets(m, c, r, what, true);
+    if (sst != TGX_OK) return sst;
     tgx::CompactParams cp{};
     cp.offs = c->d_offs;
     cp.order = c->d_order;
@@ -1540,12 +1587,20 @@
     tgx_result* r = pass.new_result(S);
     if (r->d_offs.alloc(m->device, (size_t)(S + 1) * 8) != hipSuccess)
         return fail(TGX_ERR_DEVICE, "out of device memory (result offsets)");
-    tgx_status st = run_encode_kernel(m, c, dropout, seed, pass);
+    tgx_status st = run_encode_kernel(m, c, dropout, seed, pass, r);
     if (st != TGX_OK) return st;
-    st = compact_ids(m, c, r, "encode");
-    if (st != TGX_OK) return st;
-    if (hipStreamSynchronize(m->stream) != hipSuccess)
-        return fail(TGX_ERR_DEVICE, "compact failed: %s", hipGetErrorString(hipGetLastError()));
+    if (m->last_ids_in_place) {
+        if (hipMemcpyAsync(&m->h_ctrl->err, &m->d_ctrl->err, 8, hipMemcpyDeviceToHost, m->stream) != hipSuccess ||
+            hipStreamSynchronize(m->stream) != hipSuccess)
+            return fail(TGX_ERR_DEVICE, "encode pass failed: %s", hipGetErrorString(hipGetLastError()));
+        st = check_no_path(m, c);
+        if (st != TGX_OK) return st;
+    } else {
+        st = compact_ids(m, c, r, "encode");
+        if (st != TGX_OK) return st;
+        if (hipStreamSynchronize(m->stream) != hipSuccess)
+            return fail(TGX_ERR_DEVICE, "compact failed: %s", hipGetErrorString(hipGetLastError()));
+    }
     m->last_alg_bytes = c->n_bytes + 4 * r->n_tokens + 16 * (S + 1);
     *out = pass.release_result();
     return pass.done();
@@ -4536,3 +4591,4 @@
 uint32_t tgx_model_score_values(const tgx_model* m) { return m && m->have_trie8 ? m->n_values : 0u; }
 uint32_t tgx_last_encode_hot_values(const tgx_model* m) { return m ? m->last_n_hot : 0u; }
 uint32_t tgx_last_encode_lean_items(const tgx_model* m) { return m ? m->last_lean_items : 0u; }
+int tgx_last_encode_ids_in_place(const tgx_model* m) { return (m && m->last_ids_in_place) ? 1 : 0; }
diff --git a/tokengeex_amd/csrc/trace_body.h b/tokengeex_amd/csrc/trace_body.h
--- a/tokengeex_amd/csrc/trace_body.h
+++ b/tokengeex_amd/csrc/trace_body.h
@@ -59,8 +59,8 @@
 
 template <bool CARRY> struct TraceRingEntry { using type = uint2; };
 template <> struct TraceRingEntry<true> { using type = uint4; };
-template <uint32_t LM, bool PERM, bool STAMP, bool CARRY, int K>
-__device__ __forceinline__ void trace_body(const EncodeParams& P, typename TraceRingEntry<CARRY>::type* ring) {
+template <uint32_t LM, bool PERM, bool STAMP, bool CARRY, int K, bool INPLACE = false>
+__device__ __forceinline__ void trace_body(const EncodeParams& P, typename TraceRingEntry<CARRY>::type* ring, const TraceInPlace O = TraceInPlace{nullptr, nullptr}) {
     static_assert(LM == 16 || LM == 32, "token lengths of up to 16 or 32 bytes");
     constexpr uint32_t LMASK = LM - 1u;
     constexpr int NW = (int)LM / 4;
@@ -81,27 +81,39 @@
     struct MetaRaw {
         uint64_t beg, end;
         uint32_t reach;
+        uint64_t out_end;
+        uint32_t count;
     };
     struct Meta {
         uint32_t s;
         uint64_t beg;
         uint32_t n, reach_n;
+        uint64_t out_end;
+        uint32_t count;
     };
     auto meta_request = [&](uint32_t smp) -> MetaRaw {
-        MetaRaw r{0, 0, 1u};
+        MetaRaw r{0, 0, 1u, 0, 0u};
         if (smp != kNone) {
             r.beg = P.offs[smp];
             r.end = P.offs[smp + 1];
             r.reach = P.status[smp];
+            if constexpr (INPLACE) {
+                r.out_end = O.out_offs[smp + 1];
+                r.count = P.counts[smp];
+            }
         }
         return r;
     };
     auto meta_read = [&](uint32_t smp, const MetaRaw& r) -> Meta {
-        Meta mt{smp, 0, 0, 1u};
+        Meta mt{smp, 0, 0, 1u, 0, 0u};
         if (smp != kNone) {
             mt.beg = first_u64(r.beg);
             mt.n = (uint32_t)(first_u64(r.end) - mt.beg);
             mt.reach_n = (mt.n == 0) ? 1u : (uint32_t)__builtin_amdgcn_readfirstlane((int)r.reach);
+            if constexpr (INPLACE) {
+                mt.out_end = first_u64(r.out_end);
+                mt.count = (uint32_t)__builtin_amdgcn_readfirstlane((int)r.count);
+            }
         }
         return mt;
     };
@@ -154,7 +166,8 @@
                 slot = (slot + 1u) & P.tokhash_mask;
             }
             if (!found) atomicMin(P.err_sample, (unsigned long long)((end - len) & ((1ULL << 62) - 1ULL)) | (1ULL << 62));
-            P.tmp[out] = id;
+            if constexpr (INPLACE) O.ids[out] = id;
+            else P.tmp[out] = id;
         }
         if constexpr (!CARRY) flush_out_top -= m;
         head = (head + m) & (kTraceRing - 1u);
@@ -177,8 +190,8 @@
         const uint32_t reach_n = cur.reach_n;
         const bool have = s != kNone;
         const uint8_t* __restrict__ bp = P.bp8 + (have ? bp8_base(beg, s) : 0);
-        uint32_t total = 0;
-        uint64_t out_top = beg + n;
+        uint32_t total = INPLACE ? cur.count : 0u;
+        uint64_t out_top = INPLACE ? cur.out_end : beg + n;
         flush_beg = beg;
         flush_out_top = out_top;
         int64_t q = (have && reach_n) ? (int64_t)n - 1 : (int64_t)-1;
@@ -197,9 +210,16 @@
             if (wq >= 64u) h_next = (uint32_t)bp[PERM ? bp8_perm(wq - 64u + lane) : wq - 64u + lane];
             TGX_TRACE_STAMP(1)
             int32_t qq = (int32_t)((uint32_t)q - wq);
-            const uint64_t ends = trace_hops<K>(prev, qq);
+            uint64_t ends = trace_hops<K>(prev, qq);
             q = (int64_t)wq + qq;
-            const uint32_t cnt = (uint32_t)__popcll(ends);
+            uint32_t cnt = (uint32_t)__popcll(ends);
+            if constexpr (INPLACE) {
+                const bool ov = cnt > total;
+                ends = ov ? 0ULL : ends;
+                cnt = ov ? 0u : cnt;
+                q = ov ? (int64_t)-1 : q;
+                total = ov ? 0xFFFFFFFFu : total;
+            }
             TGX_TRACE_STAMP(2)
             if ((ends >> lane) & 1ULL) {
                 const uint32_t below = __builtin_amdgcn_mbcnt_hi((uint32_t)(ends >> 32), __builtin_amdgcn_mbcnt_lo((uint32_t)ends, 0u));
@@ -212,7 +232,8 @@
                 }
             }
             fill += cnt;
-            total += cnt;
+            if constexpr (INPLACE) total -= cnt;
+            else total += cnt;
             out_top -= cnt;
             __builtin_amdgcn_wave_barrier();
             if (fill >= 64u) lookup(64u);
@@ -225,7 +246,11 @@
             if (fill) lookup(fill);
         }
         if (have && lane == 0) {
-            P.counts[s] = total;
+            if constexpr (INPLACE) {
+                if (total != 0u) atomicMin(P.err_sample, kErrCountMismatch | (unsigned long long)s);
+            } else {
+                P.counts[s] = total;
+            }
             if (!reach_n) atomicMin(P.err_sample, (unsigned long long)s);
         }
         cur = nxt;
```

Measured after the change: 72450 (median of 6 runs). 1.01x the previous value.
